# xeTaiz/vit-tf

Measured on AMD Instinct MI355X. Metric: slices/sec (ViT-S/8, 512^3 vol: feature volume + 16-query similarity), higher is better.
Workload: dtype fp16; 1 GPU; 512^3 CT-like synthetic volume (seed 0), ViT-S/8, fos 64: 1536 slices of 512x512 (N=4097) per step + 16-query similarity -> the metric's configuration (BASELINE configs[2]); engine_batch=512, weights=seeded synthetic vits8 (seed 0), parallelism=single GPU

## Files before the change

include/vittf.h:

```cpp
#ifndef VITTF_H
#define VITTF_H

#include <stddef.h>
#include <stdint.h>

#ifdef __cplusplus
extern "C" {
#endif

#define VITTF_ABI_VERSION 6

typedef enum vittf_status {
  VITTF_OK = 0,
  VITTF_ERR_INVALID_ARG = -1,
  VITTF_ERR_WORKSPACE = -2,
  VITTF_ERR_LAUNCH = -3,
  VITTF_ERR_NO_DEVICE = -4
} vittf_status;

typedef enum vittf_dtype { VITTF_BF16 = 0, VITTF_FP16 = 1 } vittf_dtype;

typedef enum vittf_axis { VITTF_AXIS_X = 0, VITTF_AXIS_Y = 1, VITTF_AXIS_Z = 2 } vittf_axis;

typedef enum vittf_sample_mode { VITTF_SAMPLE_NEAREST = 0, VITTF_SAMPLE_TRILINEAR = 1 } vittf_sample_mode;

int vittf_abi_version(void);
const char* vittf_status_string(int status);
int vittf_device_count(void);

typedef struct vittf_vit_config {
  int32_t embed_dim;
  int32_t depth;
  int32_t heads;
  int32_t patch;
  int32_t dtype;
  float   ln_eps;
  int32_t attention_fp8;
  int32_t flags;
} vittf_vit_config;
enum {
  VITTF_CFG_SEPARATE_LN = 1,
  VITTF_CFG_UNSCALED_Q = 2,
  VITTF_CFG_FP8_HEAD_SCALES = 4
};
#define VITTF_MAX_REGISTER_TOKENS 8
#define VITTF_TAIL_STEPS 112

typedef struct vittf_vit_weights {
  const float* pe_w_t;
  const float* pe_b;
  const void*  qkv_w;
  const float* qkv_b;
  const void*  proj_w;
  const float* proj_b;
  const void*  fc1_w;
  const float* fc1_b;
  const void*  fc2_w;
  const float* fc2_b;
  const void*  tail_packed;
  const void*  qkv_packed;
  const float* ln1_g;
  const float* ln1_b;
  const float* ln2_g;
  const float* ln2_b;
} vittf_vit_weights;

typedef struct vittf_pos_embed {
  const float* cls_plus_pos0;
  const float* patch_pos;
} vittf_pos_embed;

typedef struct vittf_slice_view {
  const float* vol;
  int64_t stride_slice;
  int64_t stride_row;
  int64_t stride_col;
  int32_t in_rows;
  int32_t in_cols;
  int32_t out_rows;
  int32_t out_cols;
  const float* minmax;
} vittf_slice_view;

size_t vittf_minmax_workspace_bytes(void);
int vittf_volume_minmax(const float* vol, int64_t n, float* out_minmax, void* ws, size_t ws_bytes, void* stream);

size_t vittf_vit_workspace_bytes(const vittf_vit_config* cfg, int32_t batch, int32_t tokens);

int vittf_vit_k_features(const vittf_vit_config* cfg, const vittf_vit_weights* w, const vittf_pos_embed* pos,
                         const vittf_slice_view* view, int32_t slice0, int32_t batch, int32_t qkv_part,
                         uint16_t* k_out, void* ws, size_t ws_bytes, void* stream);

int vittf_vit_qkv_features(const vittf_vit_config* cfg, const vittf_vit_weights* w, const vittf_pos_embed* pos,
                           const vittf_slice_view* view, int32_t slice0, int32_t batch, int32_t part_mask,
                           uint16_t* q_out, uint16_t* k_out, uint16_t* v_out, void* ws, size_t ws_bytes, void* stream);

int vittf_vit_qkv_features_reg(const vittf_vit_config* cfg, const vittf_vit_weights* w, const vittf_pos_embed* pos,
                               const vittf_slice_view* view, int32_t slice0, int32_t batch, int32_t part_mask,
                               const float* reg_rows, int32_t n_reg, uint16_t* q_out, uint16_t* k_out, uint16_t* v_out,
                               void* ws, size_t ws_bytes, void* stream);

typedef struct vittf_rope_table {
  const float* cos;
  const float* sin;
  int32_t patches;
} vittf_rope_table;

int vittf_vit_qkv_features_rope(const vittf_vit_config* cfg, const vittf_vit_weights* w, const vittf_pos_embed* pos,
                                const vittf_slice_view* view, int32_t slice0, int32_t batch, int32_t part_mask,
                                const float* reg_rows, int32_t n_reg, const vittf_rope_table* table, uint16_t* q_out,
                                uint16_t* k_out, uint16_t* v_out, void* ws, size_t ws_bytes, void* stream);

int vittf_vit_features(const vittf_vit_config* cfg, const vittf_vit_weights* w, const vittf_pos_embed* pos,
                       const vittf_slice_view* view, int32_t slice0, int32_t batch, int32_t part_mask, const float* reg_rows,
                       int32_t n_reg, const vittf_rope_table* table, const float* norm_g, const float* norm_b, uint16_t* q_out,
                       uint16_t* k_out, uint16_t* v_out, uint16_t* t_out, void* ws, size_t ws_bytes, void* stream);

typedef enum vittf_kernel_class {
  VITTF_KERNEL_PATCH_EMBED = 0, VITTF_KERNEL_LAYERNORM = 1,
  VITTF_KERNEL_GEMM = 2,
  VITTF_KERNEL_ATTENTION = 3, VITTF_KERNEL_MLP = 4,
  VITTF_KERNEL_GEMM_QKV = 5,
  VITTF_KERNEL_GEMM_PROJ = 6,
  VITTF_KERNEL_GEMM_FC1 = 7,
  VITTF_KERNEL_GEMM_FC2 = 8,
  VITTF_KERNEL_SIMILARITY = 9,
  VITTF_KERNEL_CLASSES = 10
} vittf_kernel_class;
int vittf_profiler_enable(int32_t class_mask);
int vittf_profiler_collect(double* ms_per_class, int64_t* launches_per_class);
const char* vittf_profiler_kernel_name(int32_t kernel_class);


int vittf_patch_embed(const vittf_vit_config* cfg, const vittf_vit_weights* w, const vittf_pos_embed* pos,
                      const vittf_slice_view* view, int32_t slice0, int32_t batch, float* tokens_out, void* stream);

int vittf_patch_embed_reg(const vittf_vit_config* cfg, const vittf_vit_weights* w, const vittf_pos_embed* pos,
                          const vittf_slice_view* view, int32_t slice0, int32_t batch, const float* reg_rows, int32_t n_reg,
                          float* tokens_out, void* stream);

int vittf_layernorm(const float* x, const float* g, const float* b, void* y, int64_t rows, int32_t d,
                    float eps, int32_t dtype, void* stream);

int vittf_token_features(const float* x, const float* norm_g, const float* norm_b, uint16_t* t_out, int32_t batch,
                         int32_t tokens, int32_t prefix, int32_t d, float eps, void* stream);

typedef enum vittf_epilogue {
  VITTF_EPI_BIAS = 0,
  VITTF_EPI_BIAS_GELU = 1,
  VITTF_EPI_BIAS_RESIDUAL = 2,
  VITTF_EPI_KFEAT = 3,
  VITTF_EPI_BIAS_QKV = 4
} vittf_epilogue;

int vittf_gemm(const void* a, const void* w, const float* bias, void* out, int64_t rows, int32_t n, int32_t k,
               int32_t epilogue, int32_t tokens, int32_t dtype, void* stream);

int vittf_gemm_kfeat_parts(const void* a, const void* w, const float* bias, int64_t rows, int32_t d, int32_t k,
                           int32_t tokens, int32_t part_mask, void* q_out, void* k_out, void* v_out, int32_t dtype,
                           void* stream);

int vittf_gemm_kfeat_parts_reg(const void* a, const void* w, const float* bias, int64_t rows, int32_t d, int32_t k,
                               int32_t tokens, int32_t n_reg, int32_t part_mask, void* q_out, void* k_out, void* v_out,
                               int32_t dtype, void* stream);

int vittf_gemm_residual_ln(const void* a, const void* w, const float* bias, float* x, int64_t rows, int32_t n, int32_t k,
                           int32_t dtype, const float* ln_g, const float* ln_b, float ln_eps, void* h, void* stream);

size_t vittf_gemm_as_workspace_bytes(void);
int vittf_gemm_as(const void* a, const void* w_packed, const float* bias, void* out, int64_t rows, int32_t n, int32_t k,
                  int32_t epilogue, int32_t dtype, void* tile_counter, void* stream);

size_t vittf_block_tail_workspace_bytes(void);
int vittf_block_tail(const void* attn_out, const void* w_packed, const float* proj_b, const float* ln2_g, const float* ln2_b,
                     const float* b1, const float* b2, float* x, int64_t rows, int32_t d, int32_t dtype, const float* ln_g,
                     const float* ln_b, float ln_eps, void* h_out, void* tile_counter, void* stream);

int vittf_rope_qk(void* qkv, int64_t rows, int32_t tokens, int32_t prefix, int32_t heads, const vittf_rope_table* table,
                  int32_t dtype, void* stream);

int vittf_attention(const void* qkv, void* out, int32_t batch, int32_t tokens, int32_t heads, int32_t dtype,
                    int32_t q_prescaled, void* stream);

int64_t vittf_attention_rescale_count(int32_t reset);

size_t vittf_attention_fp8_workspace_bytes(int32_t batch, int32_t tokens, int32_t heads);
int vittf_attention_fp8(const void* qkv, void* out, int32_t batch, int32_t tokens, int32_t heads, int32_t dtype, void* ws,
                        size_t ws_bytes, void* stream);

int vittf_gemm_qkv_fp8(const void* a, const void* w, const float* bias, void* qkv_out, int64_t rows, int32_t n, int32_t k,
                       int32_t tokens, int32_t heads, int32_t dtype, void* ws, size_t ws_bytes, void* stream);
int vittf_attention_fp8_rows(const void* qkv, void* out, int32_t batch, int32_t tokens, int32_t heads, int32_t dtype, void* ws,
                             size_t ws_bytes, void* stream);


int vittf_pool_slices(const uint16_t* k_slices, int32_t k_slice0, int32_t k_nslices, int32_t total_slices,
                      int32_t n_out, int32_t win0, int32_t nwin, int32_t f0, int32_t f1, int32_t d,
                      uint16_t* dst, int64_t dst_stride_d, int64_t dst_stride_win, int64_t dst_stride_row,
                      int64_t dst_stride_col, void* stream);

int vittf_pool_slices3d(const uint16_t* k_slices, int32_t k_slice0, int32_t k_nslices, int32_t total_slices,
                        int32_t n_out, int32_t win0, int32_t nwin, int32_t f0, int32_t f1, int32_t d,
                        uint16_t* dst, int64_t dst_stride_d, int64_t dst_stride_win, int64_t dst_stride_row,
                        int64_t dst_stride_col, int32_t o0, int32_t o1, int32_t slice_dim, void* stream);

int vittf_assemble_sum(const uint16_t* gz, const uint16_t* gy, const uint16_t* gx, int32_t nranks,
                       const int32_t chunk[3], int32_t d, int32_t n0, int32_t n1, int32_t n2, uint16_t* out,
                       void* stream);


int vittf_sample_features(const void* feat, int32_t feat_is_fp16, int32_t f, int32_t n0, int32_t n1, int32_t n2,
                          const float* rel, int32_t a, int32_t mode, const float* voxel_norm, float* out, void* stream);

int vittf_voxel_norm(const uint16_t* feat, int32_t f, int64_t nvox, float* out, void* stream);

size_t vittf_similarity_workspace_bytes(int32_t classes, int64_t nvox, int32_t annotations);

int vittf_similarity(const uint16_t* feat, int32_t f, int32_t n0, int32_t n1, int32_t n2, const float* qf,
                     const int32_t* class_start_host, int32_t classes, int32_t big_a_mean, const float* voxel_norm,
                     int32_t o0, int32_t o1, int32_t o2, uint8_t* out, void* ws, size_t ws_bytes, void* stream);

#define VITTF_QUERY_MAX_A 64
size_t vittf_similarity_query_workspace_bytes(int32_t classes, int64_t nvox, int32_t annotations, int32_t f);
int vittf_similarity_query(const uint16_t* feat, int32_t f, int32_t n0, int32_t n1, int32_t n2, const float* rel_host,
                           const int32_t* class_start_host, int32_t classes, int32_t big_a_mean, const float* voxel_norm,
                           int32_t o0, int32_t o1, int32_t o2, uint8_t* out, void* ws, size_t ws_bytes, void* stream);

int vittf_similarity_maps_f32(const void* feat, int32_t feat_is_fp16, int32_t f, int32_t n0, int32_t n1, int32_t n2,
                              const float* qf, const int32_t* class_start_host, int32_t classes, int32_t mode,
                              float exponent, const float* voxel_norm, float* maps_out, void* ws, size_t ws_bytes,
                              void* stream);

int vittf_topk_voxels(const float* maps, int32_t nmaps, int64_t nvox, int32_t k, int32_t* idx_out, void* stream);

int vittf_mean_pairwise_distance(const float* x, int32_t n, int32_t f, int32_t measure, float* dist, void* stream);

#define VITTF_GRAM_RUN 2048
#define VITTF_PCA_MAX_K 64

size_t vittf_feature_gram_workspace_bytes(int32_t f, int64_t nvox);
int vittf_feature_gram(const uint16_t* feat, int32_t f, int64_t nvox, double* gram, double* sums, void* ws, size_t ws_bytes,
                       void* stream);

int vittf_feature_project(const uint16_t* feat, int32_t f, int64_t nvox, const float* comp, const float* offset, int32_t k,
                          uint16_t* out, void* stream);

#define VITTF_KMEANS_MAX_C 64

int vittf_kmeans_assign(const uint16_t* feat, int32_t f, int64_t nvox, const float* cent, const float* half_sq, int32_t c,
                        uint8_t* labels, float* best, void* stream);

size_t vittf_kmeans_sums_workspace_bytes(int32_t f, int64_t nvox, int32_t c);
int vittf_kmeans_sums(const uint16_t* feat, int32_t f, int64_t nvox, const uint8_t* labels, int32_t c, double* sums,
                      int64_t* counts, void* ws, size_t ws_bytes, void* stream);

#define VITTF_SVM_MAX_CLASSES 8
#define VITTF_SVM_MAX_SV 65536

size_t vittf_svm_rbf_workspace_bytes(int32_t f, int32_t n_sv, int32_t classes);
int vittf_svm_rbf_decide(const uint16_t* feat, int32_t f, int64_t nvox, const uint16_t* sv, const float* pair_coef,
                         const float* intercept, int32_t n_sv, int32_t classes, float gamma, const float* voxel_norm,
                         uint8_t* labels, float* decision, void* ws, size_t ws_bytes, void* stream);

int vittf_svm_linear_decide(const uint16_t* feat, int32_t f, int64_t nvox, const float* w, const float* intercept,
                            int32_t classes, const float* voxel_norm, uint8_t* labels, float* decision, void* stream);

#define VITTF_FOREST_MAX_CLASSES 8
#define VITTF_FOREST_MAX_TREES 4096
#define VITTF_FOREST_MAX_NODES 65535
#define VITTF_FOREST_MAX_DEPTH 64
int vittf_forest_decide(const uint16_t* feat, int32_t f, int64_t nvox, const uint32_t* nodes, const uint16_t* leaf_values,
                        const uint32_t* tree_offset, int32_t trees, int32_t classes, int32_t max_depth, uint8_t* labels,
                        uint32_t* votes, void* stream);

#define VITTF_MLP_MAX_CLASSES 8
#define VITTF_MLP_MAX_LAYERS 2
#define VITTF_MLP_MAX_WIDTH 256
size_t vittf_mlp_workspace_bytes(int32_t f, const int32_t* widths, int32_t layers, int32_t classes);
int vittf_mlp_decide(const uint16_t* feat, int32_t f, int64_t nvox, const float* weights, const float* biases,
                     const int32_t* widths, int32_t layers, int32_t classes, const float* voxel_norm, uint8_t* labels,
                     float* logits, uint8_t* probs, void* workspace, size_t workspace_bytes, void* stream);

#define VITTF_KNN_MAX_K 32
#define VITTF_KNN_MAX_CLASSES 8
#define VITTF_KNN_MAX_BANK 65536
size_t vittf_knn_workspace_bytes(int32_t f, int32_t n_bank);
int vittf_knn_decide(const uint16_t* feat, int32_t f, int64_t nvox, const uint16_t* bank, const uint8_t* bank_class,
                     int32_t n_bank, int32_t classes, int32_t k, float inv_temperature, const float* voxel_norm,
                     uint8_t* labels, float* scores, int32_t* nn_index, float* nn_sim, void* ws, size_t ws_bytes,
                     void* stream);

#define VITTF_VOXFEAT_CHANNELS 11
size_t vittf_voxel_feature_stats_workspace_bytes(int32_t n0, int32_t n1, int32_t n2);
int vittf_voxel_feature_stats(const float* vol, int32_t n0, int32_t n1, int32_t n2, float vmax, double* stats, void* ws,
                              size_t ws_bytes, void* stream);
int vittf_voxel_features(const float* vol, int32_t n0, int32_t n1, int32_t n2, float vmax, const double* stats, int32_t channels,
                         const int64_t* voxel_index, int64_t v0, int64_t n, uint16_t* out, int64_t out_stride, void* stream);

int vittf_erode_mask(const uint8_t* src, int32_t n0, int32_t n1, int32_t n2, int32_t class_id, int32_t connectivity,
                     uint8_t* dst, void* stream);

size_t vittf_surface_shell_workspace_bytes(int32_t n0, int32_t n1, int32_t n2);
int vittf_surface_shell(const uint8_t* labels, int32_t n0, int32_t n1, int32_t n2, int32_t class_id, int32_t connectivity,
                        uint8_t* shell, void* ws, size_t ws_bytes, void* stream);

int vittf_confusion_matrix(const uint8_t* target, const uint8_t* pred, int64_t n, int32_t classes, int64_t* counts,
                           void* stream);

#define VITTF_CC_TILE0 4
#define VITTF_CC_TILE1 8
#define VITTF_CC_TILE2 64
size_t vittf_components_workspace_bytes(int32_t n0, int32_t n1, int32_t n2);
int vittf_label_components(const uint8_t* src, int32_t n0, int32_t n1, int32_t n2, int32_t select, int32_t connectivity,
                           int32_t* labels, void* ws, size_t ws_bytes, void* stream);

int vittf_component_sizes(const int32_t* labels, int64_t nvox, int32_t* sizes, void* stream);

int vittf_filter_components(const uint8_t* src, const int32_t* labels, const int32_t* sizes, int64_t nvox, int32_t min_size,
                            int32_t keep_label, int32_t fill, uint8_t* dst, void* stream);

#define VITTF_EDT_MAX_DIM 2048
#define VITTF_EDT_NO_SITE 2147483647
size_t vittf_edt_workspace_bytes(int32_t n0, int32_t n1, int32_t n2);
int vittf_edt_sq(const uint8_t* src, int32_t n0, int32_t n1, int32_t n2, int32_t value, int32_t mode, int32_t* d2_out,
                 int32_t* site_out, void* ws, size_t ws_bytes, void* stream);
int vittf_edt_sq_weighted(const uint8_t* src, int32_t n0, int32_t n1, int32_t n2, int32_t value, int32_t mode,
                          const double* w2_host, float* d2_out, int32_t* site_out, void* ws, size_t ws_bytes, void* stream);

#define VITTF_RENDER_MAX_DIM 2048
#define VITTF_RENDER_MAX_IMAGE 8192
#define VITTF_RENDER_MAX_CLASSES 8
int vittf_render_prepare(const float* volume, int64_t nvox, double vmin, double vmax, uint16_t* q, void* stream);
size_t vittf_render_occupancy_bytes(int32_t n0, int32_t n1, int32_t n2);
int vittf_render_occupancy(const uint16_t* q, int32_t n0, int32_t n1, int32_t n2, const float* table, const uint8_t* maps,
                           int32_t classes, int32_t m0, int32_t m1, int32_t m2, const int32_t* lo_host, uint8_t* occ,
                           void* stream);
int vittf_render(const uint16_t* q, int32_t n0, int32_t n1, int32_t n2, const float* spacing_host, const float* table,
                 const uint8_t* maps, int32_t classes, int32_t m0, int32_t m1, int32_t m2, const int32_t* lo_host,
                 const int32_t* hi_host, const float* class_rgbs_host, const uint8_t* occ, const float* camera_host,
                 int32_t width, int32_t height, float dt, const float* shade_host, float* rgba_out, void* stream);

int vittf_resize_nearest_u8(const uint8_t* src, int32_t n0, int32_t n1, int32_t n2, uint8_t* dst, int32_t o0, int32_t o1,
                            int32_t o2, int32_t equals, void* stream);

int vittf_widen_f16(const uint16_t* src, int64_t n, float* dst, void* stream);

typedef struct vittf_bilateral_params {
  double sigma_spatial;
  double lam;
  double a_diag_min;
  double cg_tol;
  int32_t cg_maxiter;
  int32_t bistochastize_iters;
  int32_t pad;
  float crop_threshold;
} vittf_bilateral_params;

size_t vittf_bilateral_workspace_bytes(int32_t o0, int32_t o1, int32_t o2, double sigma_spatial, int32_t luma_bins);

int vittf_bilateral_refine(const float* sim_in, int32_t n0, int32_t n1, int32_t n2, const float* volume, int32_t v0,
                           int32_t v1, int32_t v2, int32_t o0, int32_t o1, int32_t o2, const int32_t* luma_bin_host,
                           int32_t luma_bins, const vittf_bilateral_params* prm, float* sim_out, int32_t* info_host,
                           void* ws, size_t ws_bytes, void* stream);

int vittf_quantize_wrap_u8(const float* sim, int64_t n, uint8_t* out, float* max_scratch, void* stream);

int vittf_assign_labels(const uint8_t* sims, int32_t classes, int64_t n, const int32_t* thr_host, uint8_t* labels,
                        void* stream);

#ifdef __cplusplus
}
#endif
#endif
```

vit-tf_amd/_lib.py:

```python
import ctypes as C
import os

_HERE = os.path.dirname(os.path.abspath(__file__))
LIB_PATH = os.path.join(_HERE, 'libvittf.so')

BF16, FP16 = 0, 1
DTYPES = {'bf16': BF16, 'bfloat16': BF16, 'fp16': FP16, 'float16': FP16, 'half': FP16}
SAMPLE_MODES = {'nearest': 0, 'bilinear': 1, 'trilinear': 1}
EPI_BIAS, EPI_BIAS_GELU, EPI_BIAS_RESIDUAL, EPI_KFEAT, EPI_BIAS_QKV = 0, 1, 2, 3, 4


class VitConfig(C.Structure):
    _fields_ = [('embed_dim', C.c_int32), ('depth', C.c_int32), ('heads', C.c_int32), ('patch', C.c_int32),
                ('dtype', C.c_int32), ('ln_eps', C.c_float), ('attention_fp8', C.c_int32), ('flags', C.c_int32)]


CFG_SEPARATE_LN, CFG_UNSCALED_Q, CFG_FP8_HEAD_SCALES = 1, 2, 4


class VitWeights(C.Structure):
    _fields_ = [(n, C.c_void_p) for n in (
        'pe_w_t', 'pe_b', 'qkv_w', 'qkv_b', 'proj_w', 'proj_b', 'fc1_w', 'fc1_b', 'fc2_w', 'fc2_b', 'tail_packed', 'qkv_packed',
        'ln1_g', 'ln1_b', 'ln2_g', 'ln2_b')]


class PosEmbed(C.Structure):
    _fields_ = [('cls_plus_pos0', C.c_void_p), ('patch_pos', C.c_void_p)]


class RopeTable(C.Structure):
    _fields_ = [('cos', C.c_void_p), ('sin', C.c_void_p), ('patches', C.c_int32)]


class SliceView(C.Structure):
    _fields_ = [('vol', C.c_void_p), ('stride_slice', C.c_int64), ('stride_row', C.c_int64),
                ('stride_col', C.c_int64), ('in_rows', C.c_int32), ('in_cols', C.c_int32),
                ('out_rows', C.c_int32), ('out_cols', C.c_int32), ('minmax', C.c_void_p)]


class VittfError(RuntimeError):
    pass


class BilateralParams(C.Structure):
    _fields_ = [('sigma_spatial', C.c_double), ('lam', C.c_double), ('a_diag_min', C.c_double), ('cg_tol', C.c_double),
                ('cg_maxiter', C.c_int32), ('bistochastize_iters', C.c_int32), ('pad', C.c_int32),
                ('crop_threshold', C.c_float)]


_vp, _i32, _i64, _sz = C.c_void_p, C.c_int32, C.c_int64, C.c_size_t
_P = C.POINTER

SIGNATURES = {
    'vittf_abi_version': (C.c_int, []),
    'vittf_status_string': (C.c_char_p, [C.c_int]),
    'vittf_device_count': (C.c_int, []),
    'vittf_minmax_workspace_bytes': (_sz, []),
    'vittf_volume_minmax': (C.c_int, [_vp, _i64, _vp, _vp, _sz, _vp]),
    'vittf_vit_workspace_bytes': (_sz, [_P(VitConfig), _i32, _i32]),
    'vittf_vit_k_features': (C.c_int, [_P(VitConfig), _P(VitWeights), _P(PosEmbed), _P(SliceView), _i32, _i32, _i32,
                                       _vp, _vp, _sz, _vp]),
    'vittf_vit_qkv_features': (C.c_int, [_P(VitConfig), _P(VitWeights), _P(PosEmbed), _P(SliceView), _i32, _i32, _i32,
                                         _vp, _vp, _vp, _vp, _sz, _vp]),
    'vittf_vit_qkv_features_reg': (C.c_int, [_P(VitConfig), _P(VitWeights), _P(PosEmbed), _P(SliceView), _i32, _i32, _i32,
                                             _vp, _i32, _vp, _vp, _vp, _vp, _sz, _vp]),
    'vittf_vit_qkv_features_rope': (C.c_int, [_P(VitConfig), _P(VitWeights), _P(PosEmbed), _P(SliceView), _i32, _i32, _i32,
                                              _vp, _i32, _P(RopeTable), _vp, _vp, _vp, _vp, _sz, _vp]),
    'vittf_vit_features': (C.c_int, [_P(VitConfig), _P(VitWeights), _P(PosEmbed), _P(SliceView), _i32, _i32, _i32, _vp, _i32,
                                     _P(RopeTable), _vp, _vp, _vp, _vp, _vp, _vp, _vp, _sz, _vp]),
    'vittf_profiler_enable': (C.c_int, [_i32]),
    'vittf_profiler_collect': (C.c_int, [_P(C.c_double), _P(_i64)]),
    'vittf_profiler_kernel_name': (C.c_char_p, [_i32]),
    'vittf_patch_embed': (C.c_int, [_P(VitConfig), _P(VitWeights), _P(PosEmbed), _P(SliceView), _i32, _i32, _vp, _vp]),
    'vittf_patch_embed_reg': (C.c_int, [_P(VitConfig), _P(VitWeights), _P(PosEmbed), _P(SliceView), _i32, _i32, _vp, _i32, _vp,
                                        _vp]),
    'vittf_token_features': (C.c_int, [_vp, _vp, _vp, _vp, _i32, _i32, _i32, _i32, C.c_float, _vp]),
    'vittf_layernorm': (C.c_int, [_vp, _vp, _vp, _vp, _i64, _i32, C.c_float, _i32, _vp]),
    'vittf_gemm': (C.c_int, [_vp, _vp, _vp, _vp, _i64, _i32, _i32, _i32, _i32, _i32, _vp]),
    'vittf_gemm_kfeat_parts': (C.c_int, [_vp, _vp, _vp, _i64, _i32, _i32, _i32, _i32, _vp, _vp, _vp, _i32, _vp]),
    'vittf_gemm_kfeat_parts_reg': (C.c_int, [_vp, _vp, _vp, _i64, _i32, _i32, _i32, _i32, _i32, _vp, _vp, _vp, _i32, _vp]),
    'vittf_gemm_residual_ln': (C.c_int, [_vp, _vp, _vp, _vp, _i64, _i32, _i32, _i32, _vp, _vp, C.c_float, _vp, _vp]),
    'vittf_block_tail_workspace_bytes': (_sz, []),
    'vittf_block_tail': (C.c_int, [_vp, _vp, _vp, _vp, _vp, _vp, _vp, _vp, _i64, _i32, _i32, _vp, _vp, C.c_float, _vp, _vp, _vp]),
    'vittf_gemm_as_workspace_bytes': (_sz, []),
    'vittf_gemm_as': (C.c_int, [_vp, _vp, _vp, _vp, _i64, _i32, _i32, _i32, _i32, _vp, _vp]),
    'vittf_rope_qk': (C.c_int, [_vp, _i64, _i32, _i32, _i32, _P(RopeTable), _i32, _vp]),
    'vittf_attention': (C.c_int, [_vp, _vp, _i32, _i32, _i32, _i32, _i32, _vp]),
    'vittf_attention_rescale_count': (_i64, [_i32]),
    'vittf_attention_fp8_workspace_bytes': (_sz, [_i32, _i32, _i32]),
    'vittf_attention_fp8': (C.c_int, [_vp, _vp, _i32, _i32, _i32, _i32, _vp, _sz, _vp]),
    'vittf_gemm_qkv_fp8': (C.c_int, [_vp, _vp, _vp, _vp, _i64, _i32, _i32, _i32, _i32, _i32, _vp, _sz, _vp]),
    'vittf_attention_fp8_rows': (C.c_int, [_vp, _vp, _i32, _i32, _i32, _i32, _vp, _sz, _vp]),
    'vittf_pool_slices': (C.c_int, [_vp, _i32, _i32, _i32, _i32, _i32, _i32, _i32, _i32, _i32, _vp, _i64, _i64, _i64,
                                    _i64, _vp]),
    'vittf_pool_slices3d': (C.c_int, [_vp, _i32, _i32, _i32, _i32, _i32, _i32, _i32, _i32, _i32, _vp, _i64, _i64, _i64,
                                      _i64, _i32, _i32, _i32, _vp]),
    'vittf_assemble_sum': (C.c_int, [_vp, _vp, _vp, _i32, _P(_i32), _i32, _i32, _i32, _i32, _vp, _vp]),
    'vittf_sample_features': (C.c_int, [_vp, _i32, _i32, _i32, _i32, _i32, _vp, _i32, _i32, _vp, _vp, _vp]),
    'vittf_voxel_norm': (C.c_int, [_vp, _i32, _i64, _vp, _vp]),
    'vittf_similarity_workspace_bytes': (_sz, [_i32, _i64, _i32]),
    'vittf_similarity': (C.c_int, [_vp, _i32, _i32, _i32, _i32, _vp, _P(_i32), _i32, _i32, _vp, _i32, _i32, _i32, _vp, _vp,
                                   _sz, _vp]),
    'vittf_similarity_query_workspace_bytes': (_sz, [_i32, _i64, _i32, _i32]),
    'vittf_similarity_query': (C.c_int, [_vp, _i32, _i32, _i32, _i32, _P(C.c_float), _P(_i32), _i32, _i32, _vp, _i32, _i32, _i32,
                                         _vp, _vp, _sz, _vp]),
    'vittf_similarity_maps_f32': (C.c_int, [_vp, _i32, _i32, _i32, _i32, _i32, _vp, _P(_i32), _i32, _i32, C.c_float, _vp, _vp,
                                            _vp, _sz, _vp]),
    'vittf_feature_gram_workspace_bytes': (_sz, [_i32, _i64]),
    'vittf_feature_gram': (C.c_int, [_vp, _i32, _i64, _vp, _vp, _vp, _sz, _vp]),
    'vittf_feature_project': (C.c_int, [_vp, _i32, _i64, _vp, _vp, _i32, _vp, _vp]),
    'vittf_kmeans_assign': (C.c_int, [_vp, _i32, _i64, _vp, _vp, _i32, _vp, _vp, _vp]),
    'vittf_kmeans_sums_workspace_bytes': (_sz, [_i32, _i64, _i32]),
    'vittf_kmeans_sums': (C.c_int, [_vp, _i32, _i64, _vp, _i32, _vp, _vp, _vp, _sz, _vp]),
    'vittf_svm_rbf_workspace_bytes': (_sz, [_i32, _i32, _i32]),
    'vittf_svm_rbf_decide': (C.c_int, [_vp, _i32, _i64, _vp, _vp, _vp, _i32, _i32, C.c_float, _vp, _vp, _vp, _vp, _sz, _vp]),
    'vittf_svm_linear_decide': (C.c_int, [_vp, _i32, _i64, _vp, _vp, _i32, _vp, _vp, _vp, _vp]),
    'vittf_forest_decide': (C.c_int, [_vp, _i32, _i64, _vp, _vp, _vp, _i32, _i32, _i32, _vp, _vp, _vp]),
    'vittf_mlp_workspace_bytes': (_sz, [_i32, _P(_i32), _i32, _i32]),
    'vittf_mlp_decide': (C.c_int, [_vp, _i32, _i64, _vp, _vp, _P(_i32), _i32, _i32, _vp, _vp, _vp, _vp, _vp, _sz, _vp]),
    'vittf_knn_workspace_bytes': (_sz, [_i32, _i32]),
    'vittf_knn_decide': (C.c_int, [_vp, _i32, _i64, _vp, _vp, _i32, _i32, _i32, C.c_float, _vp, _vp, _vp, _vp, _vp, _vp, _sz, _vp]),
    'vittf_voxel_feature_stats_workspace_bytes': (_sz, [_i32, _i32, _i32]),
    'vittf_voxel_feature_stats': (C.c_int, [_vp, _i32, _i32, _i32, C.c_float, _vp, _vp, _sz, _vp]),
    'vittf_voxel_features': (C.c_int, [_vp, _i32, _i32, _i32, C.c_float, _vp, _i32, _vp, _i64, _i64, _vp, _i64, _vp]),
    'vittf_topk_voxels':(C.c_int, [_vp, _i32, _i64, _i32, _vp, _vp]),
    'vittf_mean_pairwise_distance': (C.c_int, [_vp, _i32, _i32, _i32, _vp, _vp]),
    'vittf_erode_mask': (C.c_int, [_vp, _i32, _i32, _i32, _i32, _i32, _vp, _vp]),
    'vittf_surface_shell_workspace_bytes': (_sz, [_i32, _i32, _i32]),
    'vittf_surface_shell': (C.c_int, [_vp, _i32, _i32, _i32, _i32, _i32, _vp, _vp, _sz, _vp]),
    'vittf_confusion_matrix': (C.c_int, [_vp, _vp, _i64, _i32, _vp, _vp]),
    'vittf_components_workspace_bytes': (_sz, [_i32, _i32, _i32]),
    'vittf_label_components': (C.c_int, [_vp, _i32, _i32, _i32, _i32, _i32, _vp, _vp, _sz, _vp]),
    'vittf_component_sizes': (C.c_int, [_vp, _i64, _vp, _vp]),
    'vittf_filter_components': (C.c_int, [_vp, _vp, _vp, _i64, _i32, _i32, _i32, _vp, _vp]),
    'vittf_edt_workspace_bytes': (_sz, [_i32, _i32, _i32]),
    'vittf_edt_sq': (C.c_int, [_vp, _i32, _i32, _i32, _i32, _i32, _vp, _vp, _vp, _sz, _vp]),
    'vittf_edt_sq_weighted': (C.c_int, [_vp, _i32, _i32, _i32, _i32, _i32, _P(C.c_double), _vp, _vp, _vp, _sz, _vp]),
    'vittf_render_prepare': (C.c_int, [_vp, _i64, C.c_double, C.c_double, _vp, _vp]),
    'vittf_render_occupancy_bytes': (_sz, [_i32, _i32, _i32]),
    'vittf_render_occupancy': (C.c_int, [_vp, _i32, _i32, _i32, _vp, _vp, _i32, _i32, _i32, _i32, _P(_i32), _vp, _vp]),
    'vittf_render': (C.c_int, [_vp, _i32, _i32, _i32, _P(C.c_float), _vp, _vp, _i32, _i32, _i32, _i32, _P(_i32), _P(_i32),
                               _P(C.c_float), _vp, _P(C.c_float), _i32, _i32, C.c_float, _P(C.c_float), _vp, _vp]),
    'vittf_resize_nearest_u8': (C.c_int, [_vp, _i32, _i32, _i32, _vp, _i32, _i32, _i32, _i32, _vp]),
    'vittf_widen_f16': (C.c_int, [_vp, _i64, _vp, _vp]),
    'vittf_bilateral_workspace_bytes': (_sz, [_i32, _i32, _i32, C.c_double, _i32]),
    'vittf_bilateral_refine': (C.c_int, [_vp, _i32, _i32, _i32, _vp, _i32, _i32, _i32, _i32, _i32, _i32, _P(_i32), _i32,
                                         _P(BilateralParams), _vp, _P(_i32), _vp, _sz, _vp]),
    'vittf_quantize_wrap_u8': (C.c_int, [_vp, _i64, _vp, _vp, _vp]),
    'vittf_assign_labels': (C.c_int, [_vp, _i32, _i64, _P(_i32), _vp, _vp]),
}

_lib = None


def load():
    global _lib
    if _lib is not None:
        return _lib
    if not os.path.exists(LIB_PATH):
        raise VittfError(
            f'{LIB_PATH} not found: the HIP library has not been built. Run '
            f'`python -c "import __graft_entry__ as g; g.build()"` (or `make -C vit-tf_amd/csrc`) first. '
            'There is no CPU fallback for this path.')
    lib = C.CDLL(LIB_PATH)
    for name, (res, args) in SIGNATURES.items():
        fn = getattr(lib, name)
        fn.restype, fn.argtypes = res, args
    if lib.vittf_abi_version() != ABI_VERSION:
        raise VittfError('libvittf.so ABI version mismatch; rebuild it')
    _lib = lib
    return lib


KERNEL_CLASSES = ('patch_embed', 'layernorm', 'gemm', 'attention', 'mlp', 'gemm_qkv', 'gemm_proj', 'gemm_fc1', 'gemm_fc2',
                  'similarity')
ABI_VERSION = 6
MAX_REGISTER_TOKENS = 8
QUERY_MAX_A = 64
GRAM_RUN = 2048
PCA_MAX_K = 64
KMEANS_MAX_C = 64
CC_TILE = (4, 8, 64)
SVM_MAX_CLASSES = 8
SVM_MAX_SV = 65536
FOREST_MAX_CLASSES = 8
FOREST_MAX_TREES = 4096
FOREST_MAX_NODES = 65535
FOREST_MAX_DEPTH = 64
MLP_MAX_CLASSES = 8
MLP_MAX_LAYERS = 2
MLP_MAX_WIDTH = 256
KNN_MAX_K = 32
KNN_MAX_CLASSES = 8
KNN_MAX_BANK = 65536
EDT_MAX_DIM = 2048
EDT_NO_SITE = 2 ** 31 - 1
RENDER_MAX_DIM = 2048
RENDER_MAX_IMAGE = 8192
RENDER_MAX_CLASSES = 8
VOXFEAT_CHANNELS = 11
KMEANS_SPANS = 128


def profiler_enable(on=True, classes=None):
    mask = 0
    if on:
        mask = -1 if classes is None else sum(1 << KERNEL_CLASSES.index(c) for c in classes)
    check(load().vittf_profiler_enable(mask), 'vittf_profiler_enable')


def kernel_name(kernel_class):
    return load().vittf_profiler_kernel_name(KERNEL_CLASSES.index(kernel_class)).decode()


def profiler_collect():
    ms = (C.c_double * len(KERNEL_CLASSES))()
    n = (C.c_int64 * len(KERNEL_CLASSES))()
    check(load().vittf_profiler_collect(ms, n), 'vittf_profiler_collect')
    return {k: (ms[i], n[i]) for i, k in enumerate(KERNEL_CLASSES)}


def check(rc, what=''):
    if rc != 0:
        msg = load().vittf_status_string(rc).decode()
        raise VittfError(f'{what or "vittf call"} failed: {msg} ({rc})')


def require_device():
    import torch
    lib = load()
    if not torch.cuda.is_available():
        raise VittfError('no GPU visible to PyTorch-ROCm: the vit-tf hot path runs only on MI355X (gfx950); '
                         'there is no CPU fallback')
    return lib


def stream_ptr():
    import torch
    return C.c_void_p(torch.cuda.current_stream().cuda_stream)


def ptr(t):
    return None if t is None else C.c_void_p(t.data_ptr())
```

vit-tf_amd/csrc/engine.hip:

```cpp
#include "vittf_internal.h"

#include <stdlib.h>
#include <vector>

namespace {
struct ProfRec { hipEvent_t a, b; int cls; };
unsigned g_prof_mask = 0;
std::vector<ProfRec> g_prof_recs;
std::vector<hipEvent_t> g_prof_pool;

hipEvent_t prof_event() {
  if (!g_prof_pool.empty()) { hipEvent_t e = g_prof_pool.back(); g_prof_pool.pop_back(); return e; }
  hipEvent_t e;
  (void)hipEventCreate(&e);
  return e;
}

struct WsLayout {
  size_t x, h, qkv, o, fp8, fp8_bytes, tile_ctr, total;
};

WsLayout ws_layout(int d, int64_t rows, size_t fp8_bytes = 0) {
  const int64_t rp = (rows + 127) / 128 * 128;
  WsLayout l;
  size_t off = 0;
  l.x = off;   off += align256((size_t)rp * d * 4);
  l.h = off;   off += align256((size_t)rp * d * 2);
  l.qkv = off; off += (size_t)rp * 3 * d * 2;
  l.o = off;   off += align256((size_t)rp * d * 2);
  l.fp8 = off; l.fp8_bytes = fp8_bytes; off += align256(fp8_bytes);
  l.tile_ctr = off; off += align256(vittf_block_tail_workspace_bytes());
  l.total = off;
  return l;
}

bool config_ok(const vittf_vit_config* c) {
  return c && c->embed_dim > 0 && c->embed_dim % 128 == 0 && c->embed_dim <= 1024 && c->depth >= 1 &&
         c->heads * 64 == c->embed_dim && (c->patch == 8 || c->patch == 14 || c->patch == 16) &&
         (c->dtype == VITTF_BF16 || c->dtype == VITTF_FP16) && c->ln_eps > 0.f;
}
}

void* vittf_prof_begin(int cls, void* stream) {
  if (!((g_prof_mask >> cls) & 1u)) return nullptr;
  ProfRec* r = new ProfRec;
  r->cls = cls; r->a = prof_event(); r->b = prof_event();
  (void)hipEventRecord(r->a, (hipStream_t)stream);
  return r;
}
void vittf_prof_end(void* token, void* stream) {
  ProfRec* r = (ProfRec*)token;
  (void)hipEventRecord(r->b, (hipStream_t)stream);
  g_prof_recs.push_back(*r);
  delete r;
}

extern "C" int vittf_abi_version(void) { return VITTF_ABI_VERSION; }

extern "C" const char* vittf_status_string(int status) {
  switch (status) {
    case VITTF_OK: return "ok";
    case VITTF_ERR_INVALID_ARG: return "invalid argument";
    case VITTF_ERR_WORKSPACE: return "workspace too small";
    case VITTF_ERR_LAUNCH: return "HIP launch error";
    case VITTF_ERR_NO_DEVICE: return "no gfx950 device";
    default: return "unknown status";
  }
}

extern "C" int vittf_device_count(void) {
  int n = 0;
  if (hipGetDeviceCount(&n) != hipSuccess) return 0;
  int ok = 0;
  for (int i = 0; i < n; ++i) {
    hipDeviceProp_t p;
    if (hipGetDeviceProperties(&p, i) == hipSuccess && __builtin_strstr(p.gcnArchName, "gfx950")) ++ok;
  }
  return ok;
}

extern "C" size_t vittf_vit_workspace_bytes(const vittf_vit_config* cfg, int32_t batch, int32_t tokens) {
  if (!config_ok(cfg) || batch <= 0 || tokens <= 1) return 0;
  return ws_layout(cfg->embed_dim, (int64_t)batch * tokens,
                   cfg->attention_fp8 ? vittf_attention_fp8_workspace_bytes(batch, tokens, cfg->heads) : 0).total;
}

extern "C" int vittf_vit_features(const vittf_vit_config* cfg, const vittf_vit_weights* w, const vittf_pos_embed* pos,
                                  const vittf_slice_view* view, int32_t slice0, int32_t batch, int32_t part_mask,
                                  const float* reg_rows, int32_t n_reg, const vittf_rope_table* rope, const float* norm_g,
                                  const float* norm_b, uint16_t* q_out, uint16_t* k_out, uint16_t* v_out, uint16_t* t_out,
                                  void* ws, size_t ws_bytes, void* stream) {
  if (!config_ok(cfg) || !w || !pos || !view || !ws || batch <= 0 || slice0 < 0) return VITTF_ERR_INVALID_ARG;
  if (n_reg < 0 || n_reg > VITTF_MAX_REGISTER_TOKENS || (n_reg > 0 && !reg_rows)) return VITTF_ERR_INVALID_ARG;
  if (rope && (cfg->attention_fp8 || !rope->cos || !rope->sin)) return VITTF_ERR_INVALID_ARG;
  if (part_mask <= 0 || part_mask > 15) return VITTF_ERR_INVALID_ARG;
  if (((part_mask & 1) && !q_out) || ((part_mask & 2) && !k_out) || ((part_mask & 4) && !v_out)) return VITTF_ERR_INVALID_ARG;
  const bool want_t = (part_mask & 8) != 0;
  if (want_t && (!t_out || !norm_g || !norm_b)) return VITTF_ERR_INVALID_ARG;
  if (!w->qkv_w || !w->qkv_b || !w->proj_w || !w->proj_b || !w->fc1_w || !w->fc1_b || !w->fc2_w || !w->fc2_b ||
      !w->ln1_g || !w->ln1_b || !w->ln2_g || !w->ln2_b)
    return VITTF_ERR_INVALID_ARG;
  const int d = cfg->embed_dim, p = cfg->patch, L = cfg->depth, dt = cfg->dtype;
  if (view->out_rows % p || view->out_cols % p) return VITTF_ERR_INVALID_ARG;
  const int tokens = (view->out_rows / p) * (view->out_cols / p) + 1 + n_reg;
  const int64_t rows = (int64_t)batch * tokens;
  if (rope && rope->patches != tokens - 1 - n_reg) return VITTF_ERR_INVALID_ARG;
  if (rows * (int64_t)((d == 384 && w->tail_packed) ? 3 * d : 4 * d) > 0xffffffffll) return VITTF_ERR_INVALID_ARG;
  const WsLayout lay = ws_layout(d, rows, cfg->attention_fp8 ? vittf_attention_fp8_workspace_bytes(batch, tokens, cfg->heads) : 0);
  if (ws_bytes < lay.total) return VITTF_ERR_WORKSPACE;
  if (((uintptr_t)ws & 255) != 0) return VITTF_ERR_INVALID_ARG;
  char* base = (char*)ws;
  float* X = (float*)(base + lay.x);
  void* H = base + lay.h;
  void* QKV = base + lay.qkv;
  void* O = base + lay.o;
  void* G = QKV;

  int rc;
  { ProfScope ps(VITTF_KERNEL_PATCH_EMBED, stream); rc = vittf_patch_embed_reg(cfg, w, pos, view, slice0, batch, reg_rows, n_reg, X, stream); }
  if (rc) return rc;
  const size_t esz = 2;
  const bool res_ln = !(cfg->flags & VITTF_CFG_SEPARATE_LN) && (d == 384 || d == 768);
  const int pre = (cfg->flags & VITTF_CFG_UNSCALED_Q) ? 0 : 1;
  const bool fp8_rows = !(cfg->flags & VITTF_CFG_FP8_HEAD_SCALES) && cfg->attention_fp8 && pre && d >= 768 && d % 256 == 0;
  const bool tail = d == 384 && w->tail_packed && res_ln;
  const bool qkv_as = d == 384 && w->qkv_packed && !cfg->attention_fp8;
  for (int l = 0; l < L; ++l) {
    const char* qkv_w = (const char*)w->qkv_w + (size_t)l * 3 * d * d * esz;
    if (res_ln ? l == 0 : true) {
      ProfScope ps(VITTF_KERNEL_LAYERNORM, stream);
      rc = vittf_layernorm(X, w->ln1_g + (size_t)l * d, w->ln1_b + (size_t)l * d, H, rows, d, cfg->ln_eps, dt, stream);
      if (rc) return rc;
    }
    if (l == L - 1 && (part_mask & 7)) {
      ProfScope ps(VITTF_KERNEL_GEMM, stream);
      rc = vittf_gemm_kfeat_parts_reg(H, qkv_w, w->qkv_b + (size_t)l * 3 * d, rows, d, d, tokens, n_reg, part_mask & 7, q_out,
                                      k_out, v_out, dt, stream);
      if (rc || !want_t) return rc;
    }
    const float* next_g = l == L - 1 ? norm_g : w->ln1_g + (size_t)(l + 1) * d;
    const float* next_b = l == L - 1 ? norm_b : w->ln1_b + (size_t)(l + 1) * d;
    { ProfScope ps(VITTF_KERNEL_GEMM_QKV, stream);
      if (fp8_rows)
        rc = vittf_gemm_qkv_fp8(H, qkv_w, w->qkv_b + (size_t)l * 3 * d, QKV, rows, 3 * d, d, tokens, cfg->heads, dt,
                                base + lay.fp8, lay.fp8_bytes, stream);
      else if (qkv_as)
        rc = vittf_gemm_as(H, (const char*)w->qkv_packed + (size_t)l * 3 * d * d * esz, w->qkv_b + (size_t)l * 3 * d, QKV, rows, 3 * d, d,
                           pre ? VITTF_EPI_BIAS_QKV : VITTF_EPI_BIAS, dt, base + lay.tile_ctr, stream);
      else
        rc = vittf_gemm(H, qkv_w, w->qkv_b + (size_t)l * 3 * d, QKV, rows, 3 * d, d,
                        pre ? VITTF_EPI_BIAS_QKV : VITTF_EPI_BIAS, 0, dt, stream);
      if (!rc && rope) rc = vittf_rope_qk(QKV, rows, tokens, 1 + n_reg, cfg->heads, rope, dt, stream); }
    if (rc) return rc;
    { ProfScope ps(VITTF_KERNEL_ATTENTION, stream);
      if (fp8_rows)
        rc = vittf_attention_fp8_rows(QKV, O, batch, tokens, cfg->heads, dt, base + lay.fp8, lay.fp8_bytes, stream);
      else if (cfg->attention_fp8 && pre)
        rc = vittf_attention_fp8(QKV, O, batch, tokens, cfg->heads, dt, base + lay.fp8, lay.fp8_bytes, stream);
      else
        rc = vittf_attention(QKV, O, batch, tokens, cfg->heads, dt, pre, stream); }
    if (rc) return rc;
    if (tail) {
      ProfScope ps(VITTF_KERNEL_MLP, stream);
      rc = vittf_block_tail(O, (const char*)w->tail_packed + (size_t)l * VITTF_TAIL_STEPS * 12288 * esz, w->proj_b + (size_t)l * d,
                            w->ln2_g + (size_t)l * d, w->ln2_b + (size_t)l * d, w->fc1_b + (size_t)l * 4 * d,
                            w->fc2_b + (size_t)l * d, X, rows, d, dt, next_g, next_b, cfg->ln_eps, H, base + lay.tile_ctr,
                            stream);
      if (rc) return rc;
      continue;
    }
    { ProfScope ps(VITTF_KERNEL_GEMM_PROJ, stream);
      if (res_ln)
        rc = vittf_gemm_residual_ln(O, (const char*)w->proj_w + (size_t)l * d * d * esz, w->proj_b + (size_t)l * d, X, rows, d,
                                    d, dt, w->ln2_g + (size_t)l * d, w->ln2_b + (size_t)l * d, cfg->ln_eps, H, stream);
      else
        rc = vittf_gemm(O, (const char*)w->proj_w + (size_t)l * d * d * esz, w->proj_b + (size_t)l * d, X, rows, d, d,
                        VITTF_EPI_BIAS_RESIDUAL, 0, dt, stream); }
    if (rc) return rc;
    if (!res_ln) {
      ProfScope ps(VITTF_KERNEL_LAYERNORM, stream);
      rc = vittf_layernorm(X, w->ln2_g + (size_t)l * d, w->ln2_b + (size_t)l * d, H, rows, d, cfg->ln_eps, dt, stream);
      if (rc) return rc;
    }
    { ProfScope ps(VITTF_KERNEL_GEMM_FC1, stream);
      rc = vittf_gemm(H, (const char*)w->fc1_w + (size_t)l * 4 * d * d * esz, w->fc1_b + (size_t)l * 4 * d, G, rows,
                      4 * d, d, VITTF_EPI_BIAS_GELU, 0, dt, stream); }
    if (rc) return rc;
    { ProfScope ps(VITTF_KERNEL_GEMM_FC2, stream);
      if (res_ln)
        rc = vittf_gemm_residual_ln(G, (const char*)w->fc2_w + (size_t)l * 4 * d * d * esz, w->fc2_b + (size_t)l * d, X, rows,
                                    d, 4 * d, dt, next_g, next_b, cfg->ln_eps, H, stream);
      else
        rc = vittf_gemm(G, (const char*)w->fc2_w + (size_t)l * 4 * d * d * esz, w->fc2_b + (size_t)l * d, X, rows, d,
                        4 * d, VITTF_EPI_BIAS_RESIDUAL, 0, dt, stream); }
    if (rc) return rc;
  }
  ProfScope ps(VITTF_KERNEL_LAYERNORM, stream);
  return vittf_token_features(X, norm_g, norm_b, t_out, batch, tokens, 1 + n_reg, d, cfg->ln_eps, stream);
}

extern "C" int vittf_vit_qkv_features_rope(const vittf_vit_config* cfg, const vittf_vit_weights* w, const vittf_pos_embed* pos,
                                           const vittf_slice_view* view, int32_t slice0, int32_t batch, int32_t part_mask,
                                           const float* reg_rows, int32_t n_reg, const vittf_rope_table* rope, uint16_t* q_out,
                                           uint16_t* k_out, uint16_t* v_out, void* ws, size_t ws_bytes, void* stream) {
  if (part_mask <= 0 || part_mask > 7) return VITTF_ERR_INVALID_ARG;
  return vittf_vit_features(cfg, w, pos, view, slice0, batch, part_mask, reg_rows, n_reg, rope, nullptr, nullptr, q_out, k_out,
                            v_out, nullptr, ws, ws_bytes, stream);
}

extern "C" int vittf_vit_qkv_features_reg(const vittf_vit_config* cfg, const vittf_vit_weights* w, const vittf_pos_embed* pos,
                                          const vittf_slice_view* view, int32_t slice0, int32_t batch, int32_t part_mask,
                                          const float* reg_rows, int32_t n_reg, uint16_t* q_out, uint16_t* k_out,
                                          uint16_t* v_out, void* ws, size_t ws_bytes, void* stream) {
  return vittf_vit_qkv_features_rope(cfg, w, pos, view, slice0, batch, part_mask, reg_rows, n_reg, nullptr, q_out, k_out, v_out, ws,
                                     ws_bytes, stream);
}

extern "C" int vittf_vit_qkv_features(const vittf_vit_config* cfg, const vittf_vit_weights* w, const vittf_pos_embed* pos,
                                      const vittf_slice_view* view, int32_t slice0, int32_t batch, int32_t part_mask,
                                      uint16_t* q_out, uint16_t* k_out, uint16_t* v_out, void* ws, size_t ws_bytes,
                                      void* stream) {
  return vittf_vit_qkv_features_reg(cfg, w, pos, view, slice0, batch, part_mask, nullptr, 0, q_out, k_out, v_out, ws, ws_bytes,
                                    stream);
}

extern "C" int vittf_vit_k_features(const vittf_vit_config* cfg, const vittf_vit_weights* w, const vittf_pos_embed* pos,
                                    const vittf_slice_view* view, int32_t slice0, int32_t batch, int32_t qkv_part,
                                    uint16_t* k_out, void* ws, size_t ws_bytes, void* stream) {
  if (!k_out || qkv_part < 0 || qkv_part > 2) return VITTF_ERR_INVALID_ARG;
  uint16_t* outs[3] = {nullptr, nullptr, nullptr};
  outs[qkv_part] = k_out;
  return vittf_vit_qkv_features(cfg, w, pos, view, slice0, batch, 1 << qkv_part, outs[0], outs[1], outs[2], ws, ws_bytes,
                                stream);
}

static const char* g_kernel_names[VITTF_KERNEL_CLASSES] = {};
void vittf_note_kernel(int cls, const char* name) {
  if (cls >= 0 && cls < VITTF_KERNEL_CLASSES) g_kernel_names[cls] = name;
}
extern "C" const char* vittf_profiler_kernel_name(int32_t cls) {
  return (cls >= 0 && cls < VITTF_KERNEL_CLASSES && g_kernel_names[cls]) ? g_kernel_names[cls] : "";
}

extern "C" int vittf_profiler_enable(int32_t on) {
  for (auto& r : g_prof_recs) { g_prof_pool.push_back(r.a); g_prof_pool.push_back(r.b); }
  g_prof_recs.clear();
  g_prof_mask = (unsigned)on;
  return VITTF_OK;
}

extern "C" int vittf_profiler_collect(double* ms_per_class, int64_t* launches_per_class) {
  if (!ms_per_class || !launches_per_class) return VITTF_ERR_INVALID_ARG;
  for (int i = 0; i < VITTF_KERNEL_CLASSES; ++i) { ms_per_class[i] = 0.0; launches_per_class[i] = 0; }
  for (auto& r : g_prof_recs) {
    if (hipEventSynchronize(r.b) != hipSuccess) return VITTF_ERR_LAUNCH;
    float ms = 0.f;
    if (hipEventElapsedTime(&ms, r.a, r.b) != hipSuccess) return VITTF_ERR_LAUNCH;
    ms_per_class[r.cls] += ms;
    launches_per_class[r.cls] += 1;
  }
  return VITTF_OK;
}
```

vit-tf_amd/csrc/frontend.hip:

```cpp
#include "vittf_common.h"

namespace {

constexpr int MM_BLOCKS = 1024;

__device__ __forceinline__ void wave_minmax(float& lo, float& hi) {
#pragma unroll
  for (int off = 32; off > 0; off >>= 1) {
    lo = fminf(lo, __shfl_xor(lo, off));
    hi = fmaxf(hi, __shfl_xor(hi, off));
  }
}

__device__ __forceinline__ void block_minmax(float& lo, float& hi) {
  __shared__ float s_lo[4], s_hi[4];
  wave_minmax(lo, hi);
  const int wave = threadIdx.x >> 6, lane = threadIdx.x & 63;
  if (lane == 0) { s_lo[wave] = lo; s_hi[wave] = hi; }
  __syncthreads();
  lo = fminf(fminf(s_lo[0], s_lo[1]), fminf(s_lo[2], s_lo[3]));
  hi = fmaxf(fmaxf(s_hi[0], s_hi[1]), fmaxf(s_hi[2], s_hi[3]));
}

__global__ __launch_bounds__(256) void minmax_partial(const float* __restrict__ v, int64_t n, float* __restrict__ part) {
  float lo = INFINITY, hi = -INFINITY;
  const int64_t n4 = n >> 2;
  const float4* v4 = reinterpret_cast<const float4*>(v);
  for (int64_t i = (int64_t)blockIdx.x * 256 + threadIdx.x; i < n4; i += (int64_t)gridDim.x * 256) {
    const float4 x = v4[i];
    lo = fminf(fminf(lo, x.x), fminf(fminf(x.y, x.z), x.w));
    hi = fmaxf(fmaxf(hi, x.x), fmaxf(fmaxf(x.y, x.z), x.w));
  }
  if (blockIdx.x == 0)
    for (int64_t i = (n4 << 2) + threadIdx.x; i < n; i += 256) { lo = fminf(lo, v[i]); hi = fmaxf(hi, v[i]); }
  block_minmax(lo, hi);
  if (threadIdx.x == 0) { part[2 * blockIdx.x] = lo; part[2 * blockIdx.x + 1] = hi; }
}

__global__ __launch_bounds__(256) void minmax_final(const float* __restrict__ part, int nblocks, float* __restrict__ out) {
  float lo = INFINITY, hi = -INFINITY;
  for (int i = threadIdx.x; i < nblocks; i += 256) { lo = fminf(lo, part[2 * i]); hi = fmaxf(hi, part[2 * i + 1]); }
  block_minmax(lo, hi);
  if (threadIdx.x == 0) { out[0] = lo; out[1] = hi; }
}

constexpr int TP = 32;

template <int P>
__global__ __launch_bounds__(384) void patch_embed_kernel(vittf_slice_view view, int slice0, const float* __restrict__ w_t,
                                                          const float* __restrict__ bias,
                                                          const float* __restrict__ cls_pos0,
                                                          const float* __restrict__ patch_pos, float* __restrict__ tokens_out,
                                                          int d, int f0, int f1, int nreg, const float* __restrict__ reg_rows) {
  constexpr int PP = P * P;
  __shared__ __attribute__((aligned(16))) float px[TP][PP + 4];
  const int npatch = f0 * f1;
  const int tokens = npatch + 1 + nreg;
  const int b = blockIdx.y;
  const int p0 = blockIdx.x * TP;
  const float lo = view.minmax[0], hi = view.minmax[1];
  const float range = hi - lo;
  const float sr = (float)view.in_rows / (float)view.out_rows;
  const float sc = (float)view.in_cols / (float)view.out_cols;
  const float* slice = view.vol + (int64_t)(slice0 + b) * view.stride_slice;

  for (int e = threadIdx.x; e < TP * PP; e += blockDim.x) {
    const int pl = e / PP, k = e - pl * PP;
    const int p = p0 + pl;
    float v = 0.f;
    if (p < npatch) {
      const int py = p / f1, pxx = p - py * f1;
      const int iy = py * P + k / P, ix = pxx * P + k % P;
      int ry = (int)floorf((float)iy * sr);
      int cx = (int)floorf((float)ix * sc);
      ry = ry < view.in_rows - 1 ? ry : view.in_rows - 1;
      cx = cx < view.in_cols - 1 ? cx : view.in_cols - 1;
      const float raw = slice[(int64_t)ry * view.stride_row + (int64_t)cx * view.stride_col];
      v = (raw - lo) / range;
    }
    px[pl][k] = v;
  }
  __syncthreads();

  float* out_b = tokens_out + (int64_t)b * tokens * d;
  float* out_p = out_b + (int64_t)nreg * d;
  for (int dd = threadIdx.x; dd < d; dd += blockDim.x) {
    float acc[TP];
#pragma unroll
    for (int i = 0; i < TP; ++i) acc[i] = 0.f;
    for (int k = 0; k < PP; k += 4) {
      const float w0 = w_t[(int64_t)k * d + dd], w1 = w_t[(int64_t)(k + 1) * d + dd];
      const float w2 = w_t[(int64_t)(k + 2) * d + dd], w3 = w_t[(int64_t)(k + 3) * d + dd];
#pragma unroll
      for (int i = 0; i < TP; ++i) {
        const float4 v = *reinterpret_cast<const float4*>(&px[i][k]);
        acc[i] = fmaf(v.x, w0, acc[i]);
        acc[i] = fmaf(v.y, w1, acc[i]);
        acc[i] = fmaf(v.z, w2, acc[i]);
        acc[i] = fmaf(v.w, w3, acc[i]);
      }
    }
    const float bv = bias[dd];
#pragma unroll
    for (int i = 0; i < TP; ++i) {
      const int p = p0 + i;
      if (p < npatch) out_p[(int64_t)(1 + p) * d + dd] = acc[i] + bv + patch_pos[(int64_t)p * d + dd];
    }
  }
  if (blockIdx.x == 0)
    for (int e = threadIdx.x; e < (1 + nreg) * d; e += blockDim.x) out_b[e] = e < d ? cls_pos0[e] : reg_rows[e - d];
}

constexpr int PEM_D = 384, PEM_K = 64, PEM_FRAGS = (PEM_D / 32) * (PEM_K / 16) * 2;
__global__ __launch_bounds__(512, 1) void patch_embed_mfma_kernel(vittf_slice_view view, int slice0, int batch,
                                                                  const float* __restrict__ w_t, const float* __restrict__ bias,
                                                                  const float* __restrict__ cls_pos0,
                                                                  const float* __restrict__ patch_pos,
                                                                  float* __restrict__ tokens_out, int f0, int f1, int nreg,
                                                                  const float* __restrict__ reg_rows) {
  __shared__ __attribute__((aligned(16))) unsigned short wlds[PEM_FRAGS * 512];
  const int tid = threadIdx.x, lane = tid & 63, wave = tid >> 6;
  const int h = lane >> 5, l31 = lane & 31;
  for (int it = tid; it < (PEM_FRAGS / 2) * 64; it += 512) {
    const int fr = it >> 6, ln = it & 63;
    const int ot = fr >> 2, s = fr & 3;
    const int i = ln & 31, hh = ln >> 5;
#pragma unroll
    for (int e = 0; e < 8; ++e) {
      const float v = w_t[(int64_t)(16 * s + 8 * hh + e) * PEM_D + 32 * ot + i];
      const unsigned short hi = f32_to_f16bits(v);
      const unsigned short lo = f32_to_f16bits(v - f16bits_to_f32(hi));
      wlds[((fr * 2 + 0) * 64 + ln) * 8 + e] = hi;
      wlds[((fr * 2 + 1) * 64 + ln) * 8 + e] = lo;
    }
  }
  __syncthreads();
  const int npatch = f0 * f1, tokens = npatch + 1 + nreg;
  const int64_t rows = (int64_t)batch * tokens;
  const float lo_v = view.minmax[0], range = view.minmax[1] - view.minmax[0];
  const float sr = (float)view.in_rows / (float)view.out_rows;
  const float sc = (float)view.in_cols / (float)view.out_cols;
  const int64_t ntile = (rows + 255) / 256;
  for (int64_t tile = blockIdx.x; tile < ntile; tile += gridDim.x) {
    const int64_t r = tile * 256 + wave * 32 + l31;
    const bool valid = r < rows;
    const int b = valid ? (int)(r / tokens) : 0;
    const int t = valid ? (int)(r - (int64_t)b * tokens) : 0;
    const bool patch = valid && t > nreg;
    const int p = patch ? t - 1 - nreg : 0;
    const float* crow = t == 0 ? cls_pos0 : reg_rows + (int64_t)(t - 1) * PEM_D;
    const int py = p / f1, pxx = p - py * f1;
    const float* slice = view.vol + (int64_t)(slice0 + b) * view.stride_slice;
    s16x8_t bh[4], bl[4];
#pragma unroll
    for (int s = 0; s < 4; ++s) {
      const int iy = py * 8 + 2 * s + h;
      int ry = (int)floorf((float)iy * sr);
      ry = ry < view.in_rows - 1 ? ry : view.in_rows - 1;
      unsigned short hi[8], lo[8];
#pragma unroll
      for (int e = 0; e < 8; ++e) {
        const int ix = pxx * 8 + e;
        int cx = (int)floorf((float)ix * sc);
        cx = cx < view.in_cols - 1 ? cx : view.in_cols - 1;
        float v = 0.f;
        if (patch) v = (slice[(int64_t)ry * view.stride_row + (int64_t)cx * view.stride_col] - lo_v) / range;
        hi[e] = f32_to_f16bits(v);
        lo[e] = f32_to_f16bits(v - f16bits_to_f32(hi[e]));
      }
#pragma unroll
      for (int e = 0; e < 8; ++e) { bh[s][e] = (short)hi[e]; bl[s][e] = (short)lo[e]; }
    }
    float* orow = tokens_out + r * PEM_D;
    const float* prow = patch_pos + (int64_t)p * PEM_D;
#pragma unroll 1
    for (int pass = 0; pass < 2; ++pass) {
      f32x16_t acc[6];
#pragma unroll
      for (int j = 0; j < 6; ++j)
#pragma unroll
        for (int q = 0; q < 16; ++q) acc[j][q] = 0.f;
#pragma unroll
      for (int s = 0; s < 4; ++s)
#pragma unroll
        for (int j = 0; j < 6; ++j) {
          const int fr = (6 * pass + j) * 4 + s;
          const s16x8_t ah = *reinterpret_cast<const s16x8_t*>(&wlds[((fr * 2 + 0) * 64 + lane) * 8]);
          const s16x8_t al = *reinterpret_cast<const s16x8_t*>(&wlds[((fr * 2 + 1) * 64 + lane) * 8]);
          acc[j] = mfma32<VITTF_FP16>(ah, bh[s], acc[j]);
          acc[j] = mfma32<VITTF_FP16>(al, bh[s], acc[j]);
          acc[j] = mfma32<VITTF_FP16>(ah, bl[s], acc[j]);
        }
      if (valid) {
#pragma unroll
        for (int j = 0; j < 6; ++j)
#pragma unroll
          for (int g = 0; g < 4; ++g) {
            const int c = 32 * (6 * pass + j) + 8 * g + 4 * h;
            float4 o;
            if (patch) {
              const float4 bv = *reinterpret_cast<const float4*>(bias + c);
              const float4 pv = *reinterpret_cast<const float4*>(prow + c);
              o.x = acc[j][4 * g + 0] + bv.x + pv.x; o.y = acc[j][4 * g + 1] + bv.y + pv.y;
              o.z = acc[j][4 * g + 2] + bv.z + pv.z; o.w = acc[j][4 * g + 3] + bv.w + pv.w;
            } else {
              o = *reinterpret_cast<const float4*>(crow + c);
            }
            *reinterpret_cast<float4*>(orow + c) = o;
          }
      }
    }
  }
}

constexpr int PE14_P = 14, PE14_KS = 14, PE14_GROUPS = 3, PE14_TILES = PEM_D / 32 / PE14_GROUPS;
constexpr int PE14_FRAGS = PE14_TILES * PE14_KS * 2;
__global__ __launch_bounds__(512, 1) void patch_embed14_mfma_kernel(vittf_slice_view view, int slice0, int batch,
                                                                    const float* __restrict__ w_t,
                                                                    const float* __restrict__ bias,
                                                                    const float* __restrict__ cls_pos0,
                                                                    const float* __restrict__ patch_pos,
                                                                    float* __restrict__ tokens_out, int f0, int f1, int nreg,
                                                                    const float* __restrict__ reg_rows) {
  __shared__ __attribute__((aligned(16))) unsigned short wlds[PE14_FRAGS * 512];
  const int tid = threadIdx.x, lane = tid & 63, wave = tid >> 6;
  const int h = lane >> 5, l31 = lane & 31;
  const int grp = blockIdx.x % PE14_GROUPS, wgs = gridDim.x / PE14_GROUPS;
  const int col0 = 32 * PE14_TILES * grp;
  for (int it = tid; it < (PE14_FRAGS / 2) * 64; it += 512) {
    const int fr = it >> 6, ln = it & 63;
    const int ot = fr / PE14_KS, s = fr - ot * PE14_KS;
    const int i = ln & 31, hh = ln >> 5;
#pragma unroll
    for (int e = 0; e < 8; ++e) {
      const int kc = 8 * hh + e;
      const float v = kc < PE14_P ? w_t[(int64_t)(PE14_P * s + kc) * PEM_D + col0 + 32 * ot + i] : 0.f;
      const unsigned short hi = f32_to_f16bits(v);
      const unsigned short lo = f32_to_f16bits(v - f16bits_to_f32(hi));
      wlds[((fr * 2 + 0) * 64 + ln) * 8 + e] = hi;
      wlds[((fr * 2 + 1) * 64 + ln) * 8 + e] = lo;
    }
  }
  __syncthreads();
  const int npatch = f0 * f1, tokens = npatch + 1 + nreg;
  const int64_t rows = (int64_t)batch * tokens;
  const float lo_v = view.minmax[0], range = view.minmax[1] - view.minmax[0];
  const float sr = (float)view.in_rows / (float)view.out_rows;
  const float sc = (float)view.in_cols / (float)view.out_cols;
  const int64_t ntile = (rows + 255) / 256;
  for (int64_t tile = blockIdx.x / PE14_GROUPS; tile < ntile; tile += wgs) {
    const int64_t r = tile * 256 + wave * 32 + l31;
    const bool valid = r < rows;
    const int b = valid ? (int)(r / tokens) : 0;
    const int t = valid ? (int)(r - (int64_t)b * tokens) : 0;
    const bool patch = valid && t > nreg;
    const int p = patch ? t - 1 - nreg : 0;
    const float* crow = t == 0 ? cls_pos0 : reg_rows + (int64_t)(t - 1) * PEM_D;
    const int py = p / f1, pxx = p - py * f1;
    const float* slice = view.vol + (int64_t)(slice0 + b) * view.stride_slice;
    int64_t coff[8];
#pragma unroll
    for (int e = 0; e < 8; ++e) {
      const int ix = pxx * PE14_P + 8 * h + e;
      int cx = (int)floorf((float)ix * sc);
      cx = cx < view.in_cols - 1 ? cx : view.in_cols - 1;
      coff[e] = (int64_t)cx * view.stride_col;
    }
    f32x16_t acc[PE14_TILES];
#pragma unroll
    for (int j = 0; j < PE14_TILES; ++j)
#pragma unroll
      for (int q = 0; q < 16; ++q) acc[j][q] = 0.f;
#pragma unroll 2
    for (int s = 0; s < PE14_KS; ++s) {
      const int iy = py * PE14_P + s;
      int ry = (int)floorf((float)iy * sr);
      ry = ry < view.in_rows - 1 ? ry : view.in_rows - 1;
      const float* srow = slice + (int64_t)ry * view.stride_row;
      s16x8_t bh, bl;
#pragma unroll
      for (int e = 0; e < 8; ++e) {
        float v = 0.f;
        if (patch && 8 * h + e < PE14_P) v = (srow[coff[e]] - lo_v) / range;
        const unsigned short hi = f32_to_f16bits(v);
        const unsigned short lo = f32_to_f16bits(v - f16bits_to_f32(hi));
        bh[e] = (short)hi; bl[e] = (short)lo;
      }
#pragma unroll
      for (int j = 0; j < PE14_TILES; ++j) {
        const int fr = j * PE14_KS + s;
        const s16x8_t ah = *reinterpret_cast<const s16x8_t*>(&wlds[((fr * 2 + 0) * 64 + lane) * 8]);
        const s16x8_t al = *reinterpret_cast<const s16x8_t*>(&wlds[((fr * 2 + 1) * 64 + lane) * 8]);
        acc[j] = mfma32<VITTF_FP16>(ah, bh, acc[j]);
        acc[j] = mfma32<VITTF_FP16>(al, bh, acc[j]);
        acc[j] = mfma32<VITTF_FP16>(ah, bl, acc[j]);
      }
    }
    if (valid) {
      float* orow = tokens_out + r * PEM_D;
      const float* prow = patch_pos + (int64_t)p * PEM_D;
#pragma unroll
      for (int j = 0; j < PE14_TILES; ++j)
#pragma unroll
        for (int g = 0; g < 4; ++g) {
          const int c = col0 + 32 * j + 8 * g + 4 * h;
          float4 o;
          if (patch) {
            const float4 bv = *reinterpret_cast<const float4*>(bias + c);
            const float4 pv = *reinterpret_cast<const float4*>(prow + c);
            o.x = acc[j][4 * g + 0] + bv.x + pv.x; o.y = acc[j][4 * g + 1] + bv.y + pv.y;
            o.z = acc[j][4 * g + 2] + bv.z + pv.z; o.w = acc[j][4 * g + 3] + bv.w + pv.w;
          } else {
            o = *reinterpret_cast<const float4*>(crow + c);
          }
          *reinterpret_cast<float4*>(orow + c) = o;
        }
    }
  }
}

}

extern "C" size_t vittf_minmax_workspace_bytes(void) { return 2 * MM_BLOCKS * sizeof(float); }

extern "C" int vittf_volume_minmax(const float* vol, int64_t n, float* out_minmax, void* ws, size_t ws_bytes,
                                   void* stream) {
  if (!vol || !out_minmax || !ws || n <= 0) return VITTF_ERR_INVALID_ARG;
  if (ws_bytes < vittf_minmax_workspace_bytes()) return VITTF_ERR_WORKSPACE;
  if (((uintptr_t)vol & 15) != 0) return VITTF_ERR_INVALID_ARG;
  hipStream_t st = (hipStream_t)stream;
  int64_t want = (n / 4 + 255) / 256;
  const int blocks = (int)(want < 1 ? 1 : (want > MM_BLOCKS ? MM_BLOCKS : want));
  hipLaunchKernelGGL(minmax_partial, dim3(blocks), dim3(256), 0, st, vol, n, (float*)ws);
  hipLaunchKernelGGL(minmax_final, dim3(1), dim3(256), 0, st, (const float*)ws, blocks, out_minmax);
  return vittf_check_launch();
}

extern "C" int vittf_patch_embed_reg(const vittf_vit_config* cfg, const vittf_vit_weights* w, const vittf_pos_embed* pos,
                                     const vittf_slice_view* view, int32_t slice0, int32_t batch, const float* reg_rows,
                                     int32_t n_reg, float* tokens_out, void* stream) {
  if (!cfg || !w || !pos || !view || !tokens_out || batch <= 0 || slice0 < 0) return VITTF_ERR_INVALID_ARG;
  if (n_reg < 0 || n_reg > VITTF_MAX_REGISTER_TOKENS || (n_reg > 0 && !reg_rows)) return VITTF_ERR_INVALID_ARG;
  if (!w->pe_w_t || !w->pe_b || !pos->cls_plus_pos0 || !pos->patch_pos || !view->vol || !view->minmax)
    return VITTF_ERR_INVALID_ARG;
  const int p = cfg->patch;
  if ((p != 8 && p != 14 && p != 16) || view->out_rows % p || view->out_cols % p || view->out_rows <= 0 || view->out_cols <= 0)
    return VITTF_ERR_INVALID_ARG;
  if (view->in_rows <= 0 || view->in_cols <= 0 || batch > 65535) return VITTF_ERR_INVALID_ARG;
  const int f0 = view->out_rows / p, f1 = view->out_cols / p;
  const int nblk = (f0 * f1 + TP - 1) / TP;
  hipStream_t st = (hipStream_t)stream;
  const bool aligned = (((uintptr_t)w->pe_b | (uintptr_t)pos->cls_plus_pos0 | (uintptr_t)pos->patch_pos | (uintptr_t)tokens_out |
                         (n_reg > 0 ? (uintptr_t)reg_rows : 0)) & 15) == 0;
  if (cfg->embed_dim == PEM_D && p == 8 && aligned) {
    const int cus = vittf_current_cus();
    if (cus <= 0) return VITTF_ERR_NO_DEVICE;
    const int64_t ntile = ((int64_t)batch * (f0 * f1 + 1 + n_reg) + 255) / 256;
    vittf_note_kernel(VITTF_KERNEL_PATCH_EMBED, "patch_embed_mfma_kernel");
    hipLaunchKernelGGL(patch_embed_mfma_kernel, dim3((unsigned)(ntile < cus ? ntile : cus)), dim3(512), 0, st, *view, slice0, batch,
                       w->pe_w_t, w->pe_b, pos->cls_plus_pos0, pos->patch_pos, tokens_out, f0, f1, n_reg, reg_rows);
    return vittf_check_launch();
  }
  if (cfg->embed_dim == PEM_D && p == PE14_P && aligned) {
    const int cus = vittf_current_cus();
    if (cus <= 0) return VITTF_ERR_NO_DEVICE;
    const int64_t ntile = ((int64_t)batch * (f0 * f1 + 1 + n_reg) + 255) / 256;
    const int per_group = cus / PE14_GROUPS > 0 ? cus / PE14_GROUPS : 1;
    const int wgs = (int)(ntile < per_group ? ntile : per_group);
    vittf_note_kernel(VITTF_KERNEL_PATCH_EMBED, "patch_embed14_mfma_kernel");
    hipLaunchKernelGGL(patch_embed14_mfma_kernel, dim3((unsigned)(PE14_GROUPS * wgs)), dim3(512), 0, st, *view, slice0, batch,
                       w->pe_w_t, w->pe_b, pos->cls_plus_pos0, pos->patch_pos, tokens_out, f0, f1, n_reg, reg_rows);
    return vittf_check_launch();
  }
  const int threads = cfg->embed_dim % 384 == 0 ? 384 : 256;
  if (p == 8) {
    vittf_note_kernel(VITTF_KERNEL_PATCH_EMBED, "patch_embed_kernel<8>");
    hipLaunchKernelGGL((patch_embed_kernel<8>), dim3(nblk, batch), dim3(threads), 0, st, *view, slice0, w->pe_w_t, w->pe_b,
                       pos->cls_plus_pos0, pos->patch_pos, tokens_out, cfg->embed_dim, f0, f1, n_reg, reg_rows);
  } else if (p == 14) {
    vittf_note_kernel(VITTF_KERNEL_PATCH_EMBED, "patch_embed_kernel<14>");
    hipLaunchKernelGGL((patch_embed_kernel<14>), dim3(nblk, batch), dim3(threads), 0, st, *view, slice0, w->pe_w_t, w->pe_b,
                       pos->cls_plus_pos0, pos->patch_pos, tokens_out, cfg->embed_dim, f0, f1, n_reg, reg_rows);
  } else {
    vittf_note_kernel(VITTF_KERNEL_PATCH_EMBED, "patch_embed_kernel<16>");
    hipLaunchKernelGGL((patch_embed_kernel<16>), dim3(nblk, batch), dim3(threads), 0, st, *view, slice0, w->pe_w_t, w->pe_b,
                       pos->cls_plus_pos0, pos->patch_pos, tokens_out, cfg->embed_dim, f0, f1, n_reg, reg_rows);
  }
  return vittf_check_launch();
}

extern "C" int vittf_patch_embed(const vittf_vit_config* cfg, const vittf_vit_weights* w, const vittf_pos_embed* pos,
                                 const vittf_slice_view* view, int32_t slice0, int32_t batch, float* tokens_out,
                                 void* stream) {
  return vittf_patch_embed_reg(cfg, w, pos, view, slice0, batch, nullptr, 0, tokens_out, stream);
}
```

vit-tf_amd/csrc/tail_fx.hip:

```cpp
#include "vittf_common.h"

#include <type_traits>
#include <utility>

namespace {

constexpr int D = 384, HID = 4 * D, UNITS = HID / 32;
constexpr int SB = 24576, HB = SB / 2;
constexpr int PSTEPS = D / 32;
constexpr int LAG = 4;
constexpr int MSTEPS = 2 * UNITS + LAG;
constexpr int NSEQ = PSTEPS + MSTEPS;
constexpr int NSLOT = 4, AHEAD = NSLOT - 1;
constexpr int PIECES = SB / 1024 / 4;
constexpr int WAIT0 = (AHEAD - 2) * PIECES;
constexpr int NF = 4;
constexpr int PB_OFF = NSLOT * SB;
constexpr int PBH = 4608, PB = 2 * PBH;
constexpr int STG_ROW = 144;
constexpr int AF_SLOT = 1056, AF_H = 528;
constexpr int CONST_OFF = PB_OFF + 4 * PB;
constexpr int C_B1 = 0, C_B2 = HID, C_G1 = HID + D, C_E1 = HID + 2 * D,
              C_BP = HID + 3 * D, C_G2 = HID + 4 * D, C_E2 = HID + 5 * D,
              C_N = HID + 6 * D;
constexpr int NEXT_OFF = CONST_OFF + C_N * 4;
constexpr int LDS_BYTES = NEXT_OFF + 16;
static_assert(LDS_BYTES <= 160 * 1024, "LDS");
static_assert(AHEAD >= 3, "ring depth");
static_assert(32 * STG_ROW <= PBH && 4 * AF_SLOT <= PBH, "pair buffer");

typedef __attribute__((ext_vector_type(4))) unsigned u32x4_t;
typedef __attribute__((ext_vector_type(2))) unsigned u32x2_t;
typedef __attribute__((address_space(3))) const s16x8_t* lds_frag_ptr;
typedef __attribute__((address_space(3))) const f32x4_t* lds_f4_ptr;
typedef __attribute__((address_space(3))) f32x4_t* lds_w4_ptr;
typedef __attribute__((address_space(3))) u32x4_t* lds_wu4_ptr;
typedef __attribute__((address_space(3))) u32x2_t* lds_w2_ptr;
typedef __attribute__((address_space(3))) volatile unsigned* lds_u32_ptr;

struct Ring {
  i32x4_t rsrc;
  unsigned dma_dst;
  int src0;
  int g;
  int slot;
};

__device__ __forceinline__ s16x8_t ld_frag(const unsigned (&base)[4], int f) {
  return *(lds_frag_ptr)(base[f & 3] + (f >> 2) * 4096);
}

__device__ __forceinline__ void lds_dma16_keep(i32x4_t rsrc, unsigned lds_addr, int voff, int soff) {
  asm volatile("s_mov_b32 m0, %0\n\ts_nop 0\n\tbuffer_load_dwordx4 %1, %2, %3 offen lds"
               :: "s"(lds_addr), "v"(voff), "s"(rsrc), "s"(soff) : "memory");
}

struct Gelu3 { float x, p; };
__device__ __forceinline__ void gelu_a(Gelu3& s, float x) {
  s.x = x;
  asm volatile("" : "+v"(s.x));
  s.p = fmaf(-0.000524238159f, fabsf(s.x), 0.00741911121f);
  s.p = fmaf(s.p, fabsf(s.x), -0.0526018888f);
  s.p = fmaf(s.p, fabsf(s.x), -0.459225923f);
  asm volatile("" : "+v"(s.x), "+v"(s.p));
}
__device__ __forceinline__ void gelu_b(Gelu3& s) {
  s.p = fmaf(s.p, fabsf(s.x), -1.15109742f);
  s.p = __builtin_amdgcn_exp2f(fmaf(s.p, fabsf(s.x), -1.0f));
  asm volatile("" : "+v"(s.p));
}
__device__ __forceinline__ float gelu_c(const Gelu3& s) {
  float v = fmaf(-fabsf(s.x), s.p, fmaxf(s.x, 0.f));
  asm volatile("" : "+v"(v));
  return v;
}

template <int WAITN, bool LGKM = false>
__device__ __forceinline__ void x_wait() {
  static_assert(WAITN <= 63, "vmcnt");
  if constexpr (WAITN < 0) {
    if constexpr (LGKM) asm volatile("s_waitcnt lgkmcnt(0)\n\ts_barrier" ::: "memory");
    else asm volatile("s_barrier" ::: "memory");
  } else if constexpr (LGKM) {
    asm volatile("s_waitcnt vmcnt(%0) lgkmcnt(0)\n\ts_barrier" ::"i"(WAITN) : "memory");
  } else {
    asm volatile("s_waitcnt vmcnt(%0)\n\ts_barrier" ::"i"(WAITN) : "memory");
  }
}
template <bool LGKM = false>
__device__ __forceinline__ void sync_wait() {
  if constexpr (LGKM) asm volatile("s_waitcnt lgkmcnt(0)\n\ts_barrier" ::: "memory");
  else asm volatile("s_barrier" ::: "memory");
}

__device__ __forceinline__ int ring_next(const Ring& st) { return st.g + AHEAD < NSEQ ? st.g + AHEAD : st.g + AHEAD - NSEQ; }
__device__ __forceinline__ int ring_free(const Ring& st) { return st.slot == 0 ? NSLOT - 1 : st.slot - 1; }
__device__ __forceinline__ void ring_advance(Ring& st) {
  st.g = st.g + 1 == NSEQ ? 0 : st.g + 1;
  st.slot = st.slot + 1 == NSLOT ? 0 : st.slot + 1;
}
__device__ __forceinline__ void ring_piece(const Ring& st, int i, int g_next, int slot_free) {
  const int off = st.src0 + i * 1024;
  lds_dma16_keep(st.rsrc, st.dma_dst + slot_free * SB + off, (int)((threadIdx.x & 63) * 16), g_next * SB + off);
}
__device__ __forceinline__ void rotate_bases(const Ring& st, unsigned (&base)[4]) {
  const int d_ = st.slot == NSLOT - 1 ? -(NSLOT - 1) * SB : SB;
#pragma unroll
  for (int i = 0; i < 4; ++i) {
    base[i] += d_;
    asm volatile("" : "+v"(base[i]));
  }
}

template <bool LAST, bool DMA, int NM = 12>
__device__ __forceinline__ void ring_gap(const Ring& st, unsigned (&base)[4], s16x8_t (&wf)[NF], int j, int g_next, int slot_free) {
  if (j == NM - NF && !LAST) rotate_bases(st, base);
  if (!(LAST && j >= NM - NF)) wf[j % NF] = ld_frag(base, (j + NF) % NM);
  if (DMA && j % (NM / PIECES) == NM / PIECES - 1) ring_piece(st, j / (NM / PIECES), g_next, slot_free);
}

template <int WAITN, bool LGKM = false>
__device__ __forceinline__ void x_idle_step(Ring& st) {
  x_wait<WAITN, LGKM>();
  const int g_next = ring_next(st), slot_free = ring_free(st);
#pragma unroll
  for (int i = 0; i < PIECES; ++i) ring_piece(st, i, g_next, slot_free);
  ring_advance(st);
}

template <int DT, int KH, bool GELU, bool LAST, bool LGKM>
__device__ __forceinline__ void f_step(Ring& st, unsigned (&base)[4], s16x8_t (&wf)[NF], const s16x8_t (&hf)[D / 16],
                                       f32x16_t& gacc, const f32x16_t& bias_c, const f32x16_t& gprev, u32x4_t& pk) {
  sync_wait<LGKM>();
  Gelu3 s0 = {}, s1 = {};
#pragma unroll
  for (int j = 0; j < 12; ++j) {
    gacc = mfma32<DT>(wf[j % NF], hf[12 * KH + j], (KH == 0 && j == 0) ? bias_c : gacc);
    ring_gap<LAST, false>(st, base, wf, j, 0, 0);
    if constexpr (GELU) {
      const int r = 8 * KH + 2 * (j / 3);
      if (j % 3 == 0) {
        gelu_a(s0, gprev[r]); gelu_a(s1, gprev[r + 1]);
      } else if (j % 3 == 1) {
        gelu_b(s0); gelu_b(s1);
      } else {
        const float v0 = gelu_c(s0), v1 = gelu_c(s1);
        pk[j / 3] = pack2_h16<DT>(v0, v1);
      }
    }
    __builtin_amdgcn_sched_barrier(0);
  }
  ring_advance(st);
}

template <int DT, int OH, bool LAST>
__device__ __forceinline__ void x_step(Ring& st, unsigned (&base)[4], s16x8_t (&wf)[NF], f32x16_t (&xacc)[D / 32],
                                       s16x8_t (&gf)[2], unsigned gf_addr) {
  x_wait<WAIT0>();
  const int g_next = ring_next(st), slot_free = ring_free(st);
  if constexpr (OH == 0) {
    gf[0] = *(lds_frag_ptr)(gf_addr);
    gf[1] = *(lds_frag_ptr)(gf_addr + 1024);
  }
#pragma unroll
  for (int j = 0; j < 12; ++j) {
    xacc[6 * OH + (j >> 1)] = mfma32<DT>(wf[j % NF], gf[j & 1], xacc[6 * OH + (j >> 1)]);
    ring_gap<LAST, true>(st, base, wf, j, g_next, slot_free);
    __builtin_amdgcn_sched_barrier(0);
  }
  ring_advance(st);
}

template <int DT, int WAITN, bool FIRST, bool LAST>
__device__ __forceinline__ void p_step(Ring& st, unsigned (&base)[4], s16x8_t (&wf)[NF], f32x16_t (&xacc)[D / 32],
                                       const s16x8_t (&acur)[2], s16x8_t (&anext)[2], unsigned anext_addr0, unsigned anext_addr1) {
  if constexpr (!FIRST) x_wait<WAITN>();
  const int g_next = ring_next(st), slot_free = ring_free(st);
  if constexpr (!LAST) {
    anext[0] = *(lds_frag_ptr)(anext_addr0);
    anext[1] = *(lds_frag_ptr)(anext_addr1);
  }
#pragma unroll
  for (int j = 0; j < 24; ++j) {
    xacc[j % 12] = mfma32<DT>(wf[j % NF], acur[j / 12], xacc[j % 12]);
    ring_gap<LAST, true, 24>(st, base, wf, j, g_next, slot_free);
    __builtin_amdgcn_sched_barrier(0);
  }
  ring_advance(st);
}

__device__ __forceinline__ constexpr int af_off(int s) { return (((s >> 2) & 1) ? 0 : PBH) + (s & 3) * AF_SLOT; }

struct Ctx {
  const unsigned short* abuf; const unsigned short* wpk; float* x; unsigned short* hout; unsigned* tile_ctr;
  int64_t rows; float ln_eps; int ntiles; int tile; unsigned lds0;
};
__device__ __forceinline__ unsigned uni(unsigned v) { return __builtin_amdgcn_readfirstlane(v); }
template <typename T> __device__ __forceinline__ T* uni_ptr(T* p) {
  const uint64_t v = reinterpret_cast<uint64_t>(p);
  return reinterpret_cast<T*>(((uint64_t)uni((unsigned)(v >> 32)) << 32) | uni((unsigned)v));
}
#define FX_ROLE_ENV                                                                                                       \
  const unsigned short* const abuf = uni_ptr(c.abuf);                                                                     \
  float* const x = uni_ptr(c.x);                                                                                          \
  unsigned short* const hout = uni_ptr(c.hout);                                                                           \
  unsigned* const tile_ctr = uni_ptr(c.tile_ctr);                                                                         \
  const int64_t rows = (int64_t)(((uint64_t)uni((unsigned)((uint64_t)c.rows >> 32)) << 32) | uni((unsigned)c.rows));     \
  const float ln_eps = __uint_as_float(uni(__float_as_uint(c.ln_eps)));                                                   \
  const int ntiles = (int)uni((unsigned)c.ntiles);                                                                        \
  int tile = (int)uni((unsigned)c.tile);                                                                                  \
  const unsigned lds0 = uni(c.lds0);                                                                                      \
  const int tid = threadIdx.x;                                                                                            \
  const int lane = tid & 63, wave = __builtin_amdgcn_readfirstlane(tid >> 6);                                             \
  const int rb = wave & 3;                                                                                                \
  const int h = lane >> 5, l31 = lane & 31;                                                                               \
  unsigned cl = lds0 + CONST_OFF + 16 * h;                                                                                \
  asm volatile("" : "+v"(cl));                                                                                            \
  auto cst4 = [&](int i) { return *(lds_f4_ptr)(cl + 4 * i); };             \
  const unsigned nxt = lds0 + NEXT_OFF;                                                                                   \
  Ring st;                                                                                                                \
  st.rsrc = lds_dma_rsrc(uni_ptr(c.wpk), (unsigned)(NSEQ * SB));                                                          \
  st.src0 = rb * (PIECES * 1024);                                                                                         \
  st.dma_dst = lds0;                                                                                                      \
  st.g = 0;                                                                                                               \
  st.slot = 0;                                                                                                            \
  const int aoff0 = tile_off(l31, h);                                                                                     \
  const unsigned pbuf = lds0 + PB_OFF + rb * PB;                           \
   \
  auto tile_rsrc = [&](const void* p, int64_t tile, int row_bytes) {                                                      \
    const int64_t first = tile * 128, left = rows - first;                                                                \
    const int nrows = tile < 0 || left <= 0 || !p ? 0 : left < 128 ? (int)left : 128;                                     \
    return __builtin_amdgcn_make_buffer_rsrc(const_cast<char*>(reinterpret_cast<const char*>(p)) + (nrows ? first : 0) * row_bytes, 0, \
                                             nrows * row_bytes, 0x00020000);                                              \
  };                                                                                                                      \
  (void)abuf; (void)x; (void)hout; (void)tile_ctr; (void)ln_eps; (void)ntiles; (void)l31; (void)aoff0; (void)nxt; (void)cst4; (void)tile_rsrc

template <int DT>
__device__ __attribute__((noinline)) void run_f(Ctx c) {
  FX_ROLE_ENV;
  asm volatile("s_setprio 3");
  unsigned pbl = pbuf + lane * 16;
  asm volatile("" : "+v"(pbl));
  u32x4_t fb[48];
  const int q8 = lane >> 3, c8 = lane & 7;
  __amdgpu_buffer_rsrc_t ra, rx;
  const int ao = (rb * 32 + q8) * (D * 2) + c8 * 16, xo = (rb * 32 + q8) * (D * 4) + c8 * 16;
  auto load_a = [&](int cg) {
#pragma unroll
    for (int i = 0; i < 4; ++i) fb[4 * cg + i] = __builtin_amdgcn_raw_buffer_load_b128(ra, ao + cg * 128, i * 8 * (D * 2), 0);
  };
  auto load_chunk = [&](int c) {
    const int r0 = c < 6 ? 24 + 4 * c : 4 * (c - 6);
#pragma unroll
    for (int i = 0; i < 4; ++i) fb[r0 + i] = __builtin_amdgcn_raw_buffer_load_b128(rx, xo + c * 128, i * 8 * (D * 4), 0);
  };
  const unsigned af_wr = pbuf + (c8 >> 1) * AF_SLOT + (c8 & 1) * AF_H + q8 * 16;
  auto put_a = [&](int cg) {
#pragma unroll
    for (int i = 0; i < 4; ++i) *(lds_wu4_ptr)(af_wr + af_off(4 * cg) + i * 128) = fb[4 * cg + i];
  };
  const unsigned ch_wr = pbuf + q8 * STG_ROW + c8 * 16;
  auto put_chunk = [&](int c) {
    const int r0 = c < 6 ? 24 + 4 * c : 4 * (c - 6);
#pragma unroll
    for (int i = 0; i < 4; ++i) *(lds_wu4_ptr)(ch_wr + (c & 1) * PBH + i * 8 * STG_ROW) = fb[r0 + i];
  };
  auto fetch_rows = [&](int t) {
    ra = tile_rsrc(abuf, t, D * 2);
    rx = tile_rsrc(x, t, D * 4);
#pragma unroll
    for (int cg = 0; cg < 6; ++cg) load_a(cg);
#pragma unroll
    for (int c = 0; c < 6; ++c) load_chunk(c);
    put_a(0);
  };
  fetch_rows(tile);
  asm volatile("s_waitcnt vmcnt(0)" ::: "memory");
  __syncthreads();
  while (true) {
    unsigned next_v = 0;
    if (tid == 256) next_v = atomicAdd(tile_ctr, 1u);
    unsigned base[4];
    s16x8_t hf[D / 16];
    s16x8_t wf[NF];
    f32x16_t bias_c;
    auto load_bias = [&](int at) {
#pragma unroll
      for (int q = 0; q < 4; ++q) {
        const f32x4_t bv = cst4(at + 8 * q);
        bias_c[4 * q + 0] = bv[0]; bias_c[4 * q + 1] = bv[1]; bias_c[4 * q + 2] = bv[2]; bias_c[4 * q + 3] = bv[3];
      }
    };
#pragma unroll
    for (int p = 0; p < PSTEPS; ++p) {
      sync_wait<true>();
      if (p % 2 == 0 && p / 2 + 1 < 6) put_a(p / 2 + 1);
      if (p == 0) load_chunk(6);
      if (p % 2 == 1 && p / 2 < 5) load_chunk(7 + p / 2);
      if (p == PSTEPS - 1) put_chunk(0);
      ring_advance(st);
    }
#pragma unroll
    for (int r = 0; r < 12; ++r) {
      sync_wait<true>();
      if (r + 1 < 12) put_chunk(r + 1);
    }
#pragma unroll
    for (int r = 0; r < 12; ++r) {
      sync_wait<true>();
      hf[2 * r] = *(lds_frag_ptr)(pbl + (r & 1) * PBH);
      hf[2 * r + 1] = *(lds_frag_ptr)(pbl + (r & 1) * PBH + 1024);
    }
    f32x16_t ga, gb = {};
    u32x4_t pk0 = {}, pk1 = {};
#pragma unroll
    for (int i = 0; i < 4; ++i) base[i] = lds0 + st.slot * SB + (aoff0 ^ (32 * i));
    auto put_gf = [&](int half) {
      *(lds_wu4_ptr)(pbl + half * PBH) = pk0;
      *(lds_wu4_ptr)(pbl + half * PBH + 1024) = pk1;
    };
    load_bias(C_B1);
    sync_wait<true>();
#pragma unroll
    for (int f = 0; f < NF; ++f) wf[f] = ld_frag(base, f);
#pragma unroll
    for (int j = 0; j < 12; ++j) {
      ga = mfma32<DT>(wf[j % NF], hf[j], j == 0 ? bias_c : ga);
      ring_gap<false, false>(st, base, wf, j, 0, 0);
      __builtin_amdgcn_sched_barrier(0);
    }
    ring_advance(st);
    f_step<DT, 1, false, false, false>(st, base, wf, hf, ga, bias_c, gb, pk1);
    for (int u = 1; u < UNITS - 1; u += 2) {
      load_bias(C_B1 + 32 * u);
      f_step<DT, 0, true, false, true>(st, base, wf, hf, gb, bias_c, ga, pk0);
      f_step<DT, 1, true, false, false>(st, base, wf, hf, gb, bias_c, ga, pk1);
      put_gf(0);
      load_bias(C_B1 + 32 * (u + 1));
      f_step<DT, 0, true, false, true>(st, base, wf, hf, ga, bias_c, gb, pk0);
      f_step<DT, 1, true, false, false>(st, base, wf, hf, ga, bias_c, gb, pk1);
      put_gf(1);
    }
    load_bias(C_B1 + 32 * (UNITS - 1));
    f_step<DT, 0, true, false, true>(st, base, wf, hf, gb, bias_c, ga, pk0);
    f_step<DT, 1, true, true, false>(st, base, wf, hf, gb, bias_c, ga, pk1);
    put_gf(0);
    sync_wait<true>();
    ring_advance(st);
#pragma unroll
    for (int r = 0; r < 16; r += 2) {
      const float v0 = gelu_poly(gb[r]), v1 = gelu_poly(gb[r + 1]);
      const unsigned w = pack2_h16<DT>(v0, v1);
      if (r < 8) pk0[r >> 1] = w; else pk1[(r - 8) >> 1] = w;
    }
    put_gf(1);
    sync_wait<true>(); ring_advance(st);
    sync_wait(); ring_advance(st);
    sync_wait(); ring_advance(st);
    if (tid == 256) *(lds_u32_ptr)nxt = next_v;
    asm volatile("s_waitcnt vmcnt(0) lgkmcnt(0)\n\ts_barrier" ::: "memory");
    const int next = __builtin_amdgcn_readfirstlane((int)*(lds_u32_ptr)nxt);
    if (next >= ntiles) break;
    tile = next;
    fetch_rows(tile);
  }
}

template <int DT>
__device__ __attribute__((noinline)) void run_x(Ctx c) {
  FX_ROLE_ENV;
  unsigned base[4];
  asm volatile("s_waitcnt vmcnt(0)" ::: "memory");
  __syncthreads();
  s16x8_t wf[NF];
  f32x16_t xacc[D / 32];
  while (true) {
    int ln = lane;
    asm volatile("" : "+v"(ln));
    {
#pragma unroll
      for (int ot = 0; ot < D / 32; ++ot)
#pragma unroll
        for (int q = 0; q < 4; ++q) {
          const f32x4_t bv = cst4(C_BP + 32 * ot + 8 * q);
          xacc[ot][4 * q + 0] = bv[0]; xacc[ot][4 * q + 1] = bv[1]; xacc[ot][4 * q + 2] = bv[2]; xacc[ot][4 * q + 3] = bv[3];
        }
#pragma unroll
      for (int i = 0; i < 4; ++i) base[i] = lds0 + st.slot * SB + (aoff0 ^ (32 * i));
      const unsigned af_rd = pbuf + (ln >> 5) * AF_H + (ln & 31) * 16;
      s16x8_t aa[2], ab[2];
      x_wait<-1, true>();
#pragma unroll
      for (int f = 0; f < NF; ++f) wf[f] = ld_frag(base, f);
      aa[0] = *(lds_frag_ptr)(af_rd + af_off(0));
      aa[1] = *(lds_frag_ptr)(af_rd + af_off(1));
      p_step<DT, -1, true, false>(st, base, wf, xacc, aa, ab, af_rd + af_off(2), af_rd + af_off(3));
      p_step<DT, -1, false, false>(st, base, wf, xacc, ab, aa, af_rd + af_off(4), af_rd + af_off(5));
#pragma unroll
      for (int p = 2; p < PSTEPS - 2; p += 2) {
        p_step<DT, WAIT0, false, false>(st, base, wf, xacc, aa, ab, af_rd + af_off(2 * p + 2), af_rd + af_off(2 * p + 3));
        p_step<DT, WAIT0, false, false>(st, base, wf, xacc, ab, aa, af_rd + af_off(2 * p + 4), af_rd + af_off(2 * p + 5));
      }
      p_step<DT, WAIT0, false, false>(st, base, wf, xacc, aa, ab, af_rd + af_off(2 * PSTEPS - 2), af_rd + af_off(2 * PSTEPS - 1));
      p_step<DT, WAIT0, false, true>(st, base, wf, xacc, ab, aa, 0, 0);
      const unsigned ch_rd = pbuf + (ln & 31) * STG_ROW + 16 * (ln >> 5);
#pragma unroll
      for (int r = 0; r < 12; ++r) {
        sync_wait<true>();
        f32x4_t xv[4];
#pragma unroll
        for (int g = 0; g < 4; ++g) xv[g] = *(lds_f4_ptr)(ch_rd + (r & 1) * PBH + 32 * g);
#pragma unroll
        for (int g = 0; g < 4; ++g)
#pragma unroll
          for (int e = 0; e < 4; ++e) xacc[r][4 * g + e] += xv[g][e];
      }
      float s = 0.f;
#pragma unroll
      for (int ot = 0; ot < D / 32; ++ot) {
#pragma unroll
        for (int g = 0; g < 4; ++g) s += (xacc[ot][4 * g + 0] + xacc[ot][4 * g + 1]) + (xacc[ot][4 * g + 2] + xacc[ot][4 * g + 3]);
        __builtin_amdgcn_sched_barrier(0);
      }
      {
        const auto sw = __builtin_amdgcn_permlane32_swap(__float_as_uint(s), __float_as_uint(s), false, false);
        s = __uint_as_float(sw[0]) + __uint_as_float(sw[1]);
      }
      const float mean = s / (float)D;
      float q = 0.f;
#pragma unroll
      for (int ot = 0; ot < D / 32; ++ot) {
#pragma unroll
        for (int r = 0; r < 16; ++r) { const float dv = xacc[ot][r] - mean; q += dv * dv; }
        __builtin_amdgcn_sched_barrier(0);
      }
      {
        const auto sw = __builtin_amdgcn_permlane32_swap(__float_as_uint(q), __float_as_uint(q), false, false);
        q = __uint_as_float(sw[0]) + __uint_as_float(sw[1]);
      }
      const float rstd = 1.0f / sqrtf(q / (float)D + ln_eps);
      float mean_p = mean;
      asm volatile("" : "+v"(mean_p));
      const unsigned hw_ = pbuf + ln * 16;
      f32x4_t gq[2][4], bq[2][4];
#pragma unroll
      for (int g = 0; g < 4; ++g) { gq[0][g] = cst4(C_G2 + 8 * g); bq[0][g] = cst4(C_E2 + 8 * g); }
#pragma unroll
      for (int ot = 0; ot < D / 32; ++ot) {
        if (ot + 1 < D / 32) {
#pragma unroll
          for (int g = 0; g < 4; ++g) { gq[(ot + 1) & 1][g] = cst4(C_G2 + 32 * (ot + 1) + 8 * g); bq[(ot + 1) & 1][g] = cst4(C_E2 + 32 * (ot + 1) + 8 * g); }
        }
#pragma unroll
        for (int k2 = 0; k2 < 2; ++k2) {
          u32x4_t pk;
#pragma unroll
          for (int g2_ = 0; g2_ < 2; ++g2_) {
            const int g = 2 * k2 + g2_;
            const f32x4_t gg = gq[ot & 1][g], bb = bq[ot & 1][g];
            pk[2 * g2_ + 0] = pack2_h16<DT>((xacc[ot][4 * g + 0] - mean_p) * rstd * gg[0] + bb[0], (xacc[ot][4 * g + 1] - mean_p) * rstd * gg[1] + bb[1]);
            pk[2 * g2_ + 1] = pack2_h16<DT>((xacc[ot][4 * g + 2] - mean_p) * rstd * gg[2] + bb[2], (xacc[ot][4 * g + 3] - mean_p) * rstd * gg[3] + bb[3]);
          }
          *(lds_wu4_ptr)(hw_ + (ot & 1) * PBH + k2 * 1024) = pk;
        }
        sync_wait<true>();
      }
    }
    s16x8_t gf[2];
    x_idle_step<WAIT0>(st); x_idle_step<WAIT0>(st); x_idle_step<WAIT0>(st);
    x_wait<WAIT0>();
    {
      const int g_next = ring_next(st), slot_free = ring_free(st);
#pragma unroll
      for (int i = 0; i < PIECES; ++i) ring_piece(st, i, g_next, slot_free);
      ring_advance(st);
#pragma unroll
      for (int i = 0; i < 4; ++i) base[i] = lds0 + st.slot * SB + HB + (aoff0 ^ (32 * i));
#pragma unroll
      for (int f = 0; f < NF; ++f) wf[f] = ld_frag(base, f);
    }
    const unsigned gfa = pbuf + ln * 16;
    for (int u = 0; u < UNITS - 2; u += 2) {
      x_step<DT, 0, false>(st, base, wf, xacc, gf, gfa);
      x_step<DT, 1, false>(st, base, wf, xacc, gf, gfa);
      x_step<DT, 0, false>(st, base, wf, xacc, gf, gfa + PBH);
      x_step<DT, 1, false>(st, base, wf, xacc, gf, gfa + PBH);
    }
    x_step<DT, 0, false>(st, base, wf, xacc, gf, gfa);
    x_step<DT, 1, false>(st, base, wf, xacc, gf, gfa);
    x_step<DT, 0, false>(st, base, wf, xacc, gf, gfa + PBH);
    x_step<DT, 1, true>(st, base, wf, xacc, gf, gfa + PBH);
    asm volatile("s_waitcnt vmcnt(0) lgkmcnt(0)\n\ts_barrier" ::: "memory");
    const int next = __builtin_amdgcn_readfirstlane((int)*(lds_u32_ptr)nxt);
    {
      const auto rxo = tile_rsrc(x, tile, D * 4);
      const auto rho = tile_rsrc(hout, tile, D * 2);
      int le = lane;
      asm volatile("" : "+v"(le));
      const unsigned stg_wr_e = pbuf + (le & 31) * STG_ROW + 16 * (le >> 5);
      const unsigned stg_wh = pbuf + (le & 31) * STG_ROW + 8 * (le >> 5);
      const unsigned stg_rd_e = pbuf + (le >> 3) * STG_ROW + (le & 7) * 16;
      const int xo_e = (rb * 32 + (le >> 3)) * (D * 4) + (le & 7) * 16;
      const int ho = (rb * 32 + (le >> 3)) * (D * 2) + (le & 7) * 16;
      float s = 0.f;
      {
        f32x4_t bvq[2][4];
#pragma unroll
        for (int g = 0; g < 4; ++g) bvq[0][g] = cst4(C_B2 + 8 * g);
#pragma unroll
        for (int ot = 0; ot < D / 32; ++ot) {
#pragma unroll
          for (int g = 0; g < 4; ++g) {
            const f32x4_t bv = bvq[ot & 1][g];
            f32x4_t v;
            v[0] = xacc[ot][4 * g + 0] + bv[0]; v[1] = xacc[ot][4 * g + 1] + bv[1];
            v[2] = xacc[ot][4 * g + 2] + bv[2]; v[3] = xacc[ot][4 * g + 3] + bv[3];
#pragma unroll
            for (int e = 0; e < 4; ++e) xacc[ot][4 * g + e] = v[e];
            *(lds_w4_ptr)(stg_wr_e + 32 * g) = v;
            s += (v[0] + v[1]) + (v[2] + v[3]);
          }
          __builtin_amdgcn_sched_barrier(0);
          f32x4_t rbk[4];
#pragma unroll
          for (int i = 0; i < 4; ++i) rbk[i] = *(lds_f4_ptr)(stg_rd_e + i * 8 * STG_ROW);
          if (ot + 1 < D / 32) {
#pragma unroll
            for (int g = 0; g < 4; ++g) bvq[(ot + 1) & 1][g] = cst4(C_B2 + 32 * (ot + 1) + 8 * g);
          }
          __builtin_amdgcn_sched_barrier(0);
#pragma unroll
          for (int i = 0; i < 4; ++i)
            __builtin_amdgcn_raw_buffer_store_b128(__builtin_bit_cast(u32x4_t, rbk[i]), rxo, xo_e + ot * 128, i * 8 * (D * 4), 0);
          __builtin_amdgcn_sched_barrier(0);
        }
      }
      if (hout) {
        {
          const auto sw = __builtin_amdgcn_permlane32_swap(__float_as_uint(s), __float_as_uint(s), false, false);
          s = __uint_as_float(sw[0]) + __uint_as_float(sw[1]);
        }
        const float mean = s / (float)D;
        float q = 0.f;
#pragma unroll
        for (int ot = 0; ot < D / 32; ++ot) {
#pragma unroll
          for (int r = 0; r < 16; ++r) { const float dv = xacc[ot][r] - mean; q += dv * dv; }
          __builtin_amdgcn_sched_barrier(0);
        }
        {
          const auto sw = __builtin_amdgcn_permlane32_swap(__float_as_uint(q), __float_as_uint(q), false, false);
          q = __uint_as_float(sw[0]) + __uint_as_float(sw[1]);
        }
        const float rstd = 1.0f / sqrtf(q / (float)D + ln_eps);
        float mean_p = mean;
        asm volatile("" : "+v"(mean_p));
        f32x4_t gq1[2][4], bq1[2][4];
#pragma unroll
        for (int g = 0; g < 4; ++g) { gq1[0][g] = cst4(C_G1 + 8 * g); bq1[0][g] = cst4(C_E1 + 8 * g); }
#pragma unroll
        for (int ot = 0; ot < D / 32; ++ot) {
          const int op = ot >> 1, o2 = ot & 1;
#pragma unroll
          for (int g = 0; g < 4; ++g) {
            const f32x4_t gg = gq1[ot & 1][g], bb = bq1[ot & 1][g];
            u32x2_t pk;
            pk[0] = pack2_h16<DT>((xacc[ot][4 * g + 0] - mean_p) * rstd * gg[0] + bb[0], (xacc[ot][4 * g + 1] - mean_p) * rstd * gg[1] + bb[1]);
            pk[1] = pack2_h16<DT>((xacc[ot][4 * g + 2] - mean_p) * rstd * gg[2] + bb[2], (xacc[ot][4 * g + 3] - mean_p) * rstd * gg[3] + bb[3]);
            *(lds_w2_ptr)(stg_wh + 64 * o2 + 16 * g) = pk;
          }
          __builtin_amdgcn_sched_barrier(0);
          [[maybe_unused]] f32x4_t rbk[4];
          if (o2) {
#pragma unroll
            for (int i = 0; i < 4; ++i) rbk[i] = *(lds_f4_ptr)(stg_rd_e + i * 8 * STG_ROW);
          }
          if (ot + 1 < D / 32) {
#pragma unroll
            for (int g = 0; g < 4; ++g) { gq1[(ot + 1) & 1][g] = cst4(C_G1 + 32 * (ot + 1) + 8 * g); bq1[(ot + 1) & 1][g] = cst4(C_E1 + 32 * (ot + 1) + 8 * g); }
          }
          __builtin_amdgcn_sched_barrier(0);
          if (o2) {
#pragma unroll
            for (int i = 0; i < 4; ++i)
              __builtin_amdgcn_raw_buffer_store_b128(__builtin_bit_cast(u32x4_t, rbk[i]), rho, ho + op * 128, i * 8 * (D * 2), 0);
            __builtin_amdgcn_sched_barrier(0);
          }
        }
      }
    }
    if (next >= ntiles) break;
    tile = next;
  }
}

template <int DT>
__global__ __launch_bounds__(512, 1) void tail_fx_kernel(const unsigned short* __restrict__ abuf, const unsigned short* __restrict__ wpk,
                                                         const float* __restrict__ bp, const float* __restrict__ g2, const float* __restrict__ e2,
                                                         const float* __restrict__ b1, const float* __restrict__ b2,
                                                         float* __restrict__ x, int64_t rows, const float* __restrict__ ln_g,
                                                         const float* __restrict__ ln_b, float ln_eps,
                                                         unsigned short* __restrict__ hout, int ntiles,
                                                         unsigned* __restrict__ tile_ctr) {
  __shared__ __attribute__((aligned(16))) char smem[LDS_BYTES];
  const int tid = threadIdx.x;
  const int lane = tid & 63, wave = __builtin_amdgcn_readfirstlane(tid >> 6);
  float* const cst = reinterpret_cast<float*>(smem + CONST_OFF);
  for (int i = tid; i < C_N; i += 512) {
    float v;
    if (i < C_B2) v = b1[i];
    else if (i < C_G1) v = b2[i - C_B2];
    else if (i < C_E1) v = ln_g ? ln_g[i - C_G1] : 1.f;
    else if (i < C_BP) v = ln_b ? ln_b[i - C_E1] : 0.f;
    else if (i < C_G2) v = bp[i - C_BP];
    else if (i < C_E2) v = g2[i - C_G2];
    else v = e2[i - C_E2];
    cst[i] = v;
  }
  const unsigned lds0 = (unsigned)(size_t)LDS_PTR(smem);
  const unsigned nxt = lds0 + NEXT_OFF;
  if (tid == 0) *(lds_u32_ptr)nxt = atomicAdd(tile_ctr, 1u);
  __syncthreads();
  const int tile = __builtin_amdgcn_readfirstlane((int)*(lds_u32_ptr)nxt);
  if (tile >= ntiles) return;
  if (wave < 4) {
    const i32x4_t rsrc = lds_dma_rsrc(wpk, (unsigned)(NSEQ * SB));
#pragma unroll
    for (int u = 0; u < AHEAD; ++u)
#pragma unroll
      for (int i = 0; i < PIECES; ++i)
        lds_dma16(rsrc, lds0 + wave * (PIECES * 1024) + u * SB + i * 1024, lane * 16, u * SB + wave * (PIECES * 1024) + i * 1024);
  }
  const Ctx c = {abuf, wpk, x, hout, tile_ctr, rows, ln_eps, ntiles, tile, lds0};
  if (wave >= 4) run_f<DT>(c);
  else run_x<DT>(c);
  asm volatile("s_waitcnt vmcnt(0)" ::: "memory");
}

}

extern "C" size_t vittf_block_tail_workspace_bytes(void) { return sizeof(unsigned); }

extern "C" int vittf_block_tail(const void* attn_out, const void* w_packed, const float* proj_b, const float* ln2_g,
                                const float* ln2_b, const float* b1, const float* b2, float* x, int64_t rows, int32_t d,
                                int32_t dtype, const float* ln_g, const float* ln_b, float ln_eps, void* h_out, void* tile_counter,
                                void* stream) {
  if (!attn_out || !w_packed || !proj_b || !ln2_g || !ln2_b || !b1 || !b2 || !x || rows <= 0) return VITTF_ERR_INVALID_ARG;
  if (d != D) return VITTF_ERR_INVALID_ARG;
  if ((ln_g || ln_b || h_out) && !(ln_g && ln_b && h_out)) return VITTF_ERR_INVALID_ARG;
  const int64_t tiles = (rows + 127) / 128;
  if (tiles > 0x7fffffff) return VITTF_ERR_INVALID_ARG;
  if ((((uintptr_t)attn_out | (uintptr_t)w_packed | (uintptr_t)x | (uintptr_t)h_out) & 15) != 0) return VITTF_ERR_INVALID_ARG;
  if (!tile_counter || ((uintptr_t)tile_counter & 3) != 0) return VITTF_ERR_INVALID_ARG;
  const int cus = vittf_current_cus();
  if (cus <= 0) return VITTF_ERR_NO_DEVICE;
  const unsigned grid = (unsigned)(tiles < cus ? tiles : cus);
  hipStream_t st = (hipStream_t)stream;
  unsigned* ctr = (unsigned*)tile_counter;
  if (hipMemsetAsync(ctr, 0, sizeof(unsigned), st) != hipSuccess) return VITTF_ERR_LAUNCH;
#define FX_LAUNCH(DTV)                                                                                               \
  hipLaunchKernelGGL((tail_fx_kernel<DTV>), dim3(grid), dim3(512), 0, st, (const unsigned short*)attn_out,           \
                     (const unsigned short*)w_packed, proj_b, ln2_g, ln2_b, b1, b2, x, rows, ln_g, ln_b, ln_eps,     \
                     (unsigned short*)h_out, (int)tiles, ctr)
  if (dtype == VITTF_BF16) FX_LAUNCH(VITTF_BF16);
  else if (dtype == VITTF_FP16) FX_LAUNCH(VITTF_FP16);
  else return VITTF_ERR_INVALID_ARG;
#undef FX_LAUNCH
  vittf_note_kernel(VITTF_KERNEL_MLP, "tail_fx_kernel");
  return vittf_check_launch();
}
```

vit-tf_amd/csrc/vittf_internal.h:

```cpp
#pragma once
#include "vittf_common.h"

static inline size_t align256(size_t x) { return (x + 255) & ~(size_t)255; }

static inline int64_t vittf_kfeat_out_bytes(int64_t rows, int32_t d, int32_t tokens, int32_t drop) {
  return (rows - rows / tokens * drop) * (int64_t)d * 2;
}

bool vittf_gemm_rows_covers(int32_t n, int32_t k, int64_t rows);
int vittf_gemm_rows(const void* a, const void* w, const float* bias, float* x, int64_t rows, int32_t n, int32_t k,
                    int32_t dtype, const float* ln_g, const float* ln_b, float ln_eps, void* h, hipStream_t st);

bool vittf_gemm_pp_covers(int32_t k, int32_t columns, const void* a, const void* w);
bool vittf_gemm_pp_covers_out(const void* out, int64_t kfeat_bytes);
int vittf_gemm_pp(const void* a, const void* w, const float* bias, void* out, int64_t rows, int32_t n, int32_t k,
                  int32_t epilogue, int32_t tokens, int32_t dtype, hipStream_t st);
int vittf_gemm_pp_kfeat_parts(const void* a, const void* w, const float* bias, int64_t rows, int32_t d, int32_t k,
                              int32_t tokens, int32_t n_reg, int32_t part_mask, void* const outs[3], int32_t dtype,
                              hipStream_t st, int32_t* taken);

int vittf_attention_pp64(const void* qkv, void* out, int32_t batch, int32_t tokens, int32_t heads, int32_t dtype,
                         hipStream_t st);

size_t vittf_sim_mfma_workspace_bytes(int32_t classes, int32_t annotations);
bool vittf_sim_mfma_applies(int32_t f, int32_t classes, int32_t total_a, const void* ws, size_t ws_bytes, const void* feat,
                            int64_t nvox);
int vittf_sim_mfma_maps(const unsigned short* feat, int32_t f, int64_t nvox, const float* qf, const int32_t* class_start_host,
                        int32_t classes, const float* voxel_norm, float* sim, unsigned* maxbits, void* ws, size_t ws_bytes,
                        hipStream_t st);
```

Before: 2349 slices/s.

## Fuse first LayerNorm into patch embed and skip final residual store

After: 2352 slices/s, median of 6. No clear change (+0.1%).

```diff
diff --git a/include/vittf.h b/include/vittf.h
--- a/include/vittf.h
+++ b/include/vittf.h
@@ -41,7 +41,8 @@
 enum {
   VITTF_CFG_SEPARATE_LN = 1,
   VITTF_CFG_UNSCALED_Q = 2,
-  VITTF_CFG_FP8_HEAD_SCALES = 4
+  VITTF_CFG_FP8_HEAD_SCALES = 4,
+  VITTF_CFG_SEPARATE_PASSES = 8
 };
 #define VITTF_MAX_REGISTER_TOKENS 8
 #define VITTF_TAIL_STEPS 112
@@ -139,6 +140,10 @@
                           const vittf_slice_view* view, int32_t slice0, int32_t batch, const float* reg_rows, int32_t n_reg,
                           float* tokens_out, void* stream);
 
+int vittf_patch_embed_ln(const vittf_vit_config* cfg, const vittf_vit_weights* w, const vittf_pos_embed* pos,
+                         const vittf_slice_view* view, int32_t slice0, int32_t batch, const float* reg_rows, int32_t n_reg,
+                         float* tokens_out, void* h_out, void* stream);
+
 int vittf_layernorm(const float* x, const float* g, const float* b, void* y, int64_t rows, int32_t d,
                     float eps, int32_t dtype, void* stream);
 
@@ -175,6 +180,12 @@
 int vittf_block_tail(const void* attn_out, const void* w_packed, const float* proj_b, const float* ln2_g, const float* ln2_b,
                      const float* b1, const float* b2, float* x, int64_t rows, int32_t d, int32_t dtype, const float* ln_g,
                      const float* ln_b, float ln_eps, void* h_out, void* tile_counter, void* stream);
+
+#define VITTF_TAIL_NO_X_STORE 1
+int vittf_block_tail_flags(const void* attn_out, const void* w_packed, const float* proj_b, const float* ln2_g,
+                           const float* ln2_b, const float* b1, const float* b2, float* x, int64_t rows, int32_t d, int32_t dtype,
+                           const float* ln_g, const float* ln_b, float ln_eps, void* h_out, void* tile_counter, int32_t flags,
+                           void* stream);
 
 int vittf_rope_qk(void* qkv, int64_t rows, int32_t tokens, int32_t prefix, int32_t heads, const vittf_rope_table* table,
                   int32_t dtype, void* stream);
diff --git a/vit-tf_amd/_lib.py b/vit-tf_amd/_lib.py
--- a/vit-tf_amd/_lib.py
+++ b/vit-tf_amd/_lib.py
@@ -15,7 +15,8 @@
                 ('dtype', C.c_int32), ('ln_eps', C.c_float), ('attention_fp8', C.c_int32), ('flags', C.c_int32)]
 
 
-CFG_SEPARATE_LN, CFG_UNSCALED_Q, CFG_FP8_HEAD_SCALES = 1, 2, 4
+CFG_SEPARATE_LN, CFG_UNSCALED_Q, CFG_FP8_HEAD_SCALES, CFG_SEPARATE_PASSES = 1, 2, 4, 8
+TAIL_NO_X_STORE = 1
 
 
 class VitWeights(C.Structure):
@@ -74,6 +75,8 @@
     'vittf_patch_embed': (C.c_int, [_P(VitConfig), _P(VitWeights), _P(PosEmbed), _P(SliceView), _i32, _i32, _vp, _vp]),
     'vittf_patch_embed_reg': (C.c_int, [_P(VitConfig), _P(VitWeights), _P(PosEmbed), _P(SliceView), _i32, _i32, _vp, _i32, _vp,
                                         _vp]),
+    'vittf_patch_embed_ln': (C.c_int, [_P(VitConfig), _P(VitWeights), _P(PosEmbed), _P(SliceView), _i32, _i32, _vp, _i32, _vp, _vp,
+                                       _vp]),
     'vittf_token_features': (C.c_int, [_vp, _vp, _vp, _vp, _i32, _i32, _i32, _i32, C.c_float, _vp]),
     'vittf_layernorm': (C.c_int, [_vp, _vp, _vp, _vp, _i64, _i32, C.c_float, _i32, _vp]),
     'vittf_gemm': (C.c_int, [_vp, _vp, _vp, _vp, _i64, _i32, _i32, _i32, _i32, _i32, _vp]),
@@ -82,6 +85,8 @@
     'vittf_gemm_residual_ln': (C.c_int, [_vp, _vp, _vp, _vp, _i64, _i32, _i32, _i32, _vp, _vp, C.c_float, _vp, _vp]),
     'vittf_block_tail_workspace_bytes': (_sz, []),
     'vittf_block_tail': (C.c_int, [_vp, _vp, _vp, _vp, _vp, _vp, _vp, _vp, _i64, _i32, _i32, _vp, _vp, C.c_float, _vp, _vp, _vp]),
+    'vittf_block_tail_flags': (C.c_int, [_vp, _vp, _vp, _vp, _vp, _vp, _vp, _vp, _i64, _i32, _i32, _vp, _vp, C.c_float, _vp, _vp, _i32,
+                                         _vp]),
     'vittf_gemm_as_workspace_bytes': (_sz, []),
     'vittf_gemm_as': (C.c_int, [_vp, _vp, _vp, _vp, _i64, _i32, _i32, _i32, _i32, _vp, _vp]),
     'vittf_rope_qk': (C.c_int, [_vp, _i64, _i32, _i32, _i32, _P(RopeTable), _i32, _vp]),
diff --git a/vit-tf_amd/csrc/engine.hip b/vit-tf_amd/csrc/engine.hip
--- a/vit-tf_amd/csrc/engine.hip
+++ b/vit-tf_amd/csrc/engine.hip
@@ -116,18 +116,22 @@
   void* O = base + lay.o;
   void* G = QKV;
 
-  int rc;
-  { ProfScope ps(VITTF_KERNEL_PATCH_EMBED, stream); rc = vittf_patch_embed_reg(cfg, w, pos, view, slice0, batch, reg_rows, n_reg, X, stream); }
-  if (rc) return rc;
   const size_t esz = 2;
   const bool res_ln = !(cfg->flags & VITTF_CFG_SEPARATE_LN) && (d == 384 || d == 768);
   const int pre = (cfg->flags & VITTF_CFG_UNSCALED_Q) ? 0 : 1;
   const bool fp8_rows = !(cfg->flags & VITTF_CFG_FP8_HEAD_SCALES) && cfg->attention_fp8 && pre && d >= 768 && d % 256 == 0;
   const bool tail = d == 384 && w->tail_packed && res_ln;
   const bool qkv_as = d == 384 && w->qkv_packed && !cfg->attention_fp8;
+  const bool passes = !(cfg->flags & VITTF_CFG_SEPARATE_PASSES) && !want_t;
+  const bool embed_ln = passes && tail && qkv_as && vittf_patch_embed_covers_ln(cfg, w, pos, reg_rows, n_reg, X, H);
+  int rc;
+  { ProfScope ps(VITTF_KERNEL_PATCH_EMBED, stream);
+    rc = embed_ln ? vittf_patch_embed_ln(cfg, w, pos, view, slice0, batch, reg_rows, n_reg, X, H, stream)
+                  : vittf_patch_embed_reg(cfg, w, pos, view, slice0, batch, reg_rows, n_reg, X, stream); }
+  if (rc) return rc;
   for (int l = 0; l < L; ++l) {
     const char* qkv_w = (const char*)w->qkv_w + (size_t)l * 3 * d * d * esz;
-    if (res_ln ? l == 0 : true) {
+    if (res_ln ? l == 0 && !embed_ln : true) {
       ProfScope ps(VITTF_KERNEL_LAYERNORM, stream);
       rc = vittf_layernorm(X, w->ln1_g + (size_t)l * d, w->ln1_b + (size_t)l * d, H, rows, d, cfg->ln_eps, dt, stream);
       if (rc) return rc;
@@ -161,11 +165,12 @@
         rc = vittf_attention(QKV, O, batch, tokens, cfg->heads, dt, pre, stream); }
     if (rc) return rc;
     if (tail) {
+      const int tail_flags = (passes && l == L - 2) ? VITTF_TAIL_NO_X_STORE : 0;
       ProfScope ps(VITTF_KERNEL_MLP, stream);
-      rc = vittf_block_tail(O, (const char*)w->tail_packed + (size_t)l * VITTF_TAIL_STEPS * 12288 * esz, w->proj_b + (size_t)l * d,
-                            w->ln2_g + (size_t)l * d, w->ln2_b + (size_t)l * d, w->fc1_b + (size_t)l * 4 * d,
-                            w->fc2_b + (size_t)l * d, X, rows, d, dt, next_g, next_b, cfg->ln_eps, H, base + lay.tile_ctr,
-                            stream);
+      rc = vittf_block_tail_flags(O, (const char*)w->tail_packed + (size_t)l * VITTF_TAIL_STEPS * 12288 * esz,
+                                  w->proj_b + (size_t)l * d, w->ln2_g + (size_t)l * d, w->ln2_b + (size_t)l * d,
+                                  w->fc1_b + (size_t)l * 4 * d, w->fc2_b + (size_t)l * d, X, rows, d, dt, next_g, next_b,
+                                  cfg->ln_eps, H, base + lay.tile_ctr, tail_flags, stream);
       if (rc) return rc;
       continue;
     }
diff --git a/vit-tf_amd/csrc/frontend.hip b/vit-tf_amd/csrc/frontend.hip
--- a/vit-tf_amd/csrc/frontend.hip
+++ b/vit-tf_amd/csrc/frontend.hip
@@ -1,4 +1,4 @@
-#include "vittf_common.h"
+#include "vittf_internal.h"
 
 namespace {
 
@@ -111,14 +111,61 @@
     for (int e = threadIdx.x; e < (1 + nreg) * d; e += blockDim.x) out_b[e] = e < d ? cls_pos0[e] : reg_rows[e - d];
 }
 
-constexpr int PEM_D = 384, PEM_K = 64, PEM_FRAGS = (PEM_D / 32) * (PEM_K / 16) * 2;
+constexpr int PEM_D = 384, PEM_K = 64, PEM_FRAGS = (PEM_D / 32) * (PEM_K / 16) * 2, PEM_OT = PEM_D / 32;
+
+template <typename F> __device__ __forceinline__ float row_tree_sum(F f4) {
+#pragma clang fp contract(off)
+  float t[16];
+#pragma unroll
+  for (int m = 0; m < 16; ++m) t[m] = ((0.f + f4(m)) + f4(m + 32)) + (0.f + f4(m + 16));
+#pragma unroll
+  for (int w = 8; w >= 1; w >>= 1)
+#pragma unroll
+    for (int m = 0; m < w; ++m) t[m] = t[m] + t[m + w];
+  return t[0] + __shfl_xor(t[0], 32);
+}
+
+template <int DT>
+__device__ __forceinline__ void row_layernorm(const f32x16_t (&v)[PEM_OT], int h, const float* __restrict__ g,
+                                              const float* __restrict__ b, float eps, unsigned short* __restrict__ yrow,
+                                              bool store) {
+#pragma clang fp contract(off)
+  const float s = row_tree_sum([&](int m) {
+    const int ot = m >> 2, q = 4 * (m & 3);
+    return (v[ot][q + 0] + v[ot][q + 1]) + (v[ot][q + 2] + v[ot][q + 3]);
+  });
+  const float mean = s / (float)PEM_D;
+  const float qs = row_tree_sum([&](int m) {
+    const int ot = m >> 2, q = 4 * (m & 3);
+    const float a0 = v[ot][q + 0] - mean, a1 = v[ot][q + 1] - mean, a2 = v[ot][q + 2] - mean, a3 = v[ot][q + 3] - mean;
+    return __builtin_fmaf(a0, a0, a1 * a1) + __builtin_fmaf(a2, a2, a3 * a3);
+  });
+  const float rstd = 1.0f / sqrtf(qs / (float)PEM_D + eps);
+  if (!store) return;
+#pragma unroll
+  for (int ot = 0; ot < PEM_OT; ++ot)
+#pragma unroll
+    for (int q = 0; q < 16; q += 4) {
+      const int c = 32 * ot + 2 * q + 4 * h;
+      const float4 gg = *reinterpret_cast<const float4*>(g + c), bb = *reinterpret_cast<const float4*>(b + c);
+      uint2 pk;
+      pk.x = pack2_h16<DT>(__builtin_fmaf((v[ot][q + 0] - mean) * rstd, gg.x, bb.x), __builtin_fmaf((v[ot][q + 1] - mean) * rstd, gg.y, bb.y));
+      pk.y = pack2_h16<DT>(__builtin_fmaf((v[ot][q + 2] - mean) * rstd, gg.z, bb.z), __builtin_fmaf((v[ot][q + 3] - mean) * rstd, gg.w, bb.w));
+      *reinterpret_cast<uint2*>(yrow + c) = pk;
+    }
+}
+
+template <int LN>
 __global__ __launch_bounds__(512, 1) void patch_embed_mfma_kernel(vittf_slice_view view, int slice0, int batch,
                                                                   const float* __restrict__ w_t, const float* __restrict__ bias,
                                                                   const float* __restrict__ cls_pos0,
                                                                   const float* __restrict__ patch_pos,
                                                                   float* __restrict__ tokens_out, int f0, int f1, int nreg,
-                                                                  const float* __restrict__ reg_rows) {
+                                                                  const float* __restrict__ reg_rows,
+                                                                  const float* __restrict__ ln_g, const float* __restrict__ ln_b,
+                                                                  float ln_eps, unsigned short* __restrict__ h_out) {
   __shared__ __attribute__((aligned(16))) unsigned short wlds[PEM_FRAGS * 512];
+  constexpr int TILES = LN >= 0 ? PEM_OT : PEM_OT / 2;
   const int tid = threadIdx.x, lane = tid & 63, wave = tid >> 6;
   const int h = lane >> 5, l31 = lane & 31;
   for (int it = tid; it < (PEM_FRAGS / 2) * 64; it += 512) {
@@ -173,43 +220,45 @@
     }
     float* orow = tokens_out + r * PEM_D;
     const float* prow = patch_pos + (int64_t)p * PEM_D;
+    f32x16_t acc[TILES];
 #pragma unroll 1
-    for (int pass = 0; pass < 2; ++pass) {
-      f32x16_t acc[6];
-#pragma unroll
-      for (int j = 0; j < 6; ++j)
+    for (int pass = 0; pass < PEM_OT / TILES; ++pass) {
+#pragma unroll
+      for (int j = 0; j < TILES; ++j)
 #pragma unroll
         for (int q = 0; q < 16; ++q) acc[j][q] = 0.f;
 #pragma unroll
       for (int s = 0; s < 4; ++s)
 #pragma unroll
-        for (int j = 0; j < 6; ++j) {
-          const int fr = (6 * pass + j) * 4 + s;
+        for (int j = 0; j < TILES; ++j) {
+          const int fr = (TILES * pass + j) * 4 + s;
           const s16x8_t ah = *reinterpret_cast<const s16x8_t*>(&wlds[((fr * 2 + 0) * 64 + lane) * 8]);
           const s16x8_t al = *reinterpret_cast<const s16x8_t*>(&wlds[((fr * 2 + 1) * 64 + lane) * 8]);
           acc[j] = mfma32<VITTF_FP16>(ah, bh[s], acc[j]);
           acc[j] = mfma32<VITTF_FP16>(al, bh[s], acc[j]);
           acc[j] = mfma32<VITTF_FP16>(ah, bl[s], acc[j]);
         }
-      if (valid) {
-#pragma unroll
-        for (int j = 0; j < 6; ++j)
+      if (valid || LN >= 0) {
+#pragma unroll
+        for (int j = 0; j < TILES; ++j)
 #pragma unroll
           for (int g = 0; g < 4; ++g) {
-            const int c = 32 * (6 * pass + j) + 8 * g + 4 * h;
-            float4 o;
+            const int c = 32 * (TILES * pass + j) + 8 * g + 4 * h;
+            float4 o = make_float4(0.f, 0.f, 0.f, 0.f);
             if (patch) {
               const float4 bv = *reinterpret_cast<const float4*>(bias + c);
               const float4 pv = *reinterpret_cast<const float4*>(prow + c);
               o.x = acc[j][4 * g + 0] + bv.x + pv.x; o.y = acc[j][4 * g + 1] + bv.y + pv.y;
               o.z = acc[j][4 * g + 2] + bv.z + pv.z; o.w = acc[j][4 * g + 3] + bv.w + pv.w;
-            } else {
+            } else if (valid) {
               o = *reinterpret_cast<const float4*>(crow + c);
             }
-            *reinterpret_cast<float4*>(orow + c) = o;
+            if (valid) *reinterpret_cast<float4*>(orow + c) = o;
+            if constexpr (LN >= 0) { acc[j][4 * g + 0] = o.x; acc[j][4 * g + 1] = o.y; acc[j][4 * g + 2] = o.z; acc[j][4 * g + 3] = o.w; }
           }
       }
     }
+    if constexpr (LN >= 0) row_layernorm<LN>(acc, h, ln_g, ln_b, ln_eps, h_out + r * PEM_D, valid);
   }
 }
 
@@ -336,9 +385,10 @@
   return vittf_check_launch();
 }
 
-extern "C" int vittf_patch_embed_reg(const vittf_vit_config* cfg, const vittf_vit_weights* w, const vittf_pos_embed* pos,
-                                     const vittf_slice_view* view, int32_t slice0, int32_t batch, const float* reg_rows,
-                                     int32_t n_reg, float* tokens_out, void* stream) {
+static int patch_embed(const vittf_vit_config* cfg, const vittf_vit_weights* w, const vittf_pos_embed* pos,
+                       const vittf_slice_view* view, int32_t slice0, int32_t batch, const float* reg_rows, int32_t n_reg,
+                       float* tokens_out, const float* ln_g, const float* ln_b, float ln_eps, int32_t ln_dtype, void* h_out,
+                       void* stream) {
   if (!cfg || !w || !pos || !view || !tokens_out || batch <= 0 || slice0 < 0) return VITTF_ERR_INVALID_ARG;
   if (n_reg < 0 || n_reg > VITTF_MAX_REGISTER_TOKENS || (n_reg > 0 && !reg_rows)) return VITTF_ERR_INVALID_ARG;
   if (!w->pe_w_t || !w->pe_b || !pos->cls_plus_pos0 || !pos->patch_pos || !view->vol || !view->minmax)
@@ -356,11 +406,19 @@
     const int cus = vittf_current_cus();
     if (cus <= 0) return VITTF_ERR_NO_DEVICE;
     const int64_t ntile = ((int64_t)batch * (f0 * f1 + 1 + n_reg) + 255) / 256;
+    const dim3 grid((unsigned)(ntile < cus ? ntile : cus));
     vittf_note_kernel(VITTF_KERNEL_PATCH_EMBED, "patch_embed_mfma_kernel");
-    hipLaunchKernelGGL(patch_embed_mfma_kernel, dim3((unsigned)(ntile < cus ? ntile : cus)), dim3(512), 0, st, *view, slice0, batch,
-                       w->pe_w_t, w->pe_b, pos->cls_plus_pos0, pos->patch_pos, tokens_out, f0, f1, n_reg, reg_rows);
+#define PEM_LAUNCH(LN)                                                                                                           \
+  hipLaunchKernelGGL((patch_embed_mfma_kernel<LN>), grid, dim3(512), 0, st, *view, slice0, batch, w->pe_w_t, w->pe_b,           \
+                     pos->cls_plus_pos0, pos->patch_pos, tokens_out, f0, f1, n_reg, reg_rows, ln_g, ln_b, ln_eps,               \
+                     (unsigned short*)h_out)
+    if (!h_out) PEM_LAUNCH(-1);
+    else if (ln_dtype == VITTF_BF16) PEM_LAUNCH(VITTF_BF16);
+    else PEM_LAUNCH(VITTF_FP16);
+#undef PEM_LAUNCH
     return vittf_check_launch();
   }
+  if (h_out) return VITTF_ERR_INVALID_ARG;
   if (cfg->embed_dim == PEM_D && p == PE14_P && aligned) {
     const int cus = vittf_current_cus();
     if (cus <= 0) return VITTF_ERR_NO_DEVICE;
@@ -389,6 +447,30 @@
   return vittf_check_launch();
 }
 
+extern "C" int vittf_patch_embed_reg(const vittf_vit_config* cfg, const vittf_vit_weights* w, const vittf_pos_embed* pos,
+                                     const vittf_slice_view* view, int32_t slice0, int32_t batch, const float* reg_rows,
+                                     int32_t n_reg, float* tokens_out, void* stream) {
+  return patch_embed(cfg, w, pos, view, slice0, batch, reg_rows, n_reg, tokens_out, nullptr, nullptr, 0.f, 0, nullptr, stream);
+}
+
+bool vittf_patch_embed_covers_ln(const vittf_vit_config* cfg, const vittf_vit_weights* w, const vittf_pos_embed* pos,
+                                 const float* reg_rows, int32_t n_reg, const float* tokens_out, const void* h_out) {
+  if (!cfg || !w || !pos) return false;
+  return cfg->embed_dim == PEM_D && cfg->patch == 8 &&
+         (((uintptr_t)w->pe_b | (uintptr_t)pos->cls_plus_pos0 | (uintptr_t)pos->patch_pos | (uintptr_t)tokens_out | (uintptr_t)h_out |
+           (uintptr_t)w->ln1_g | (uintptr_t)w->ln1_b | (n_reg > 0 ? (uintptr_t)reg_rows : 0)) & 15) == 0;
+}
+
+extern "C" int vittf_patch_embed_ln(const vittf_vit_config* cfg, const vittf_vit_weights* w, const vittf_pos_embed* pos,
+                                    const vittf_slice_view* view, int32_t slice0, int32_t batch, const float* reg_rows,
+                                    int32_t n_reg, float* tokens_out, void* h_out, void* stream) {
+  if (!cfg || !w || !h_out || !w->ln1_g || !w->ln1_b) return VITTF_ERR_INVALID_ARG;
+  if (cfg->dtype != VITTF_BF16 && cfg->dtype != VITTF_FP16) return VITTF_ERR_INVALID_ARG;
+  if (!vittf_patch_embed_covers_ln(cfg, w, pos, reg_rows, n_reg, tokens_out, h_out)) return VITTF_ERR_INVALID_ARG;
+  return patch_embed(cfg, w, pos, view, slice0, batch, reg_rows, n_reg, tokens_out, (const float*)w->ln1_g, (const float*)w->ln1_b,
+                     cfg->ln_eps, cfg->dtype, h_out, stream);
+}
+
 extern "C" int vittf_patch_embed(const vittf_vit_config* cfg, const vittf_vit_weights* w, const vittf_pos_embed* pos,
                                  const vittf_slice_view* view, int32_t slice0, int32_t batch, float* tokens_out,
                                  void* stream) {
diff --git a/vit-tf_amd/csrc/tail_fx.hip b/vit-tf_amd/csrc/tail_fx.hip
--- a/vit-tf_amd/csrc/tail_fx.hip
+++ b/vit-tf_amd/csrc/tail_fx.hip
@@ -366,7 +366,7 @@
   }
 }
 
-template <int DT>
+template <int DT, bool STORE_X>
 __device__ __attribute__((noinline)) void run_x(Ctx c) {
   FX_ROLE_ENV;
   unsigned base[4];
@@ -503,7 +503,7 @@
       const int xo_e = (rb * 32 + (le >> 3)) * (D * 4) + (le & 7) * 16;
       const int ho = (rb * 32 + (le >> 3)) * (D * 2) + (le & 7) * 16;
       float s = 0.f;
-      {
+      if constexpr (STORE_X) {
         f32x4_t bvq[2][4];
 #pragma unroll
         for (int g = 0; g < 4; ++g) bvq[0][g] = cst4(C_B2 + 8 * g);
@@ -532,6 +532,28 @@
 #pragma unroll
           for (int i = 0; i < 4; ++i)
             __builtin_amdgcn_raw_buffer_store_b128(__builtin_bit_cast(u32x4_t, rbk[i]), rxo, xo_e + ot * 128, i * 8 * (D * 4), 0);
+          __builtin_amdgcn_sched_barrier(0);
+        }
+      } else {
+        f32x4_t bvq[2][4];
+#pragma unroll
+        for (int g = 0; g < 4; ++g) bvq[0][g] = cst4(C_B2 + 8 * g);
+#pragma unroll
+        for (int ot = 0; ot < D / 32; ++ot) {
+          if (ot + 1 < D / 32) {
+#pragma unroll
+            for (int g = 0; g < 4; ++g) bvq[(ot + 1) & 1][g] = cst4(C_B2 + 32 * (ot + 1) + 8 * g);
+          }
+#pragma unroll
+          for (int g = 0; g < 4; ++g) {
+            const f32x4_t bv = bvq[ot & 1][g];
+            f32x4_t v;
+            v[0] = xacc[ot][4 * g + 0] + bv[0]; v[1] = xacc[ot][4 * g + 1] + bv[1];
+            v[2] = xacc[ot][4 * g + 2] + bv[2]; v[3] = xacc[ot][4 * g + 3] + bv[3];
+#pragma unroll
+            for (int e = 0; e < 4; ++e) xacc[ot][4 * g + e] = v[e];
+            s += (v[0] + v[1]) + (v[2] + v[3]);
+          }
           __builtin_amdgcn_sched_barrier(0);
         }
       }
@@ -594,14 +616,14 @@
   }
 }
 
-template <int DT>
-__global__ __launch_bounds__(512, 1) void tail_fx_kernel(const unsigned short* __restrict__ abuf, const unsigned short* __restrict__ wpk,
-                                                         const float* __restrict__ bp, const float* __restrict__ g2, const float* __restrict__ e2,
-                                                         const float* __restrict__ b1, const float* __restrict__ b2,
-                                                         float* __restrict__ x, int64_t rows, const float* __restrict__ ln_g,
-                                                         const float* __restrict__ ln_b, float ln_eps,
-                                                         unsigned short* __restrict__ hout, int ntiles,
-                                                         unsigned* __restrict__ tile_ctr) {
+#define FX_KERNEL_ARGS                                                                                                   \
+  const unsigned short *__restrict__ abuf, const unsigned short *__restrict__ wpk, const float *__restrict__ bp,         \
+      const float *__restrict__ g2, const float *__restrict__ e2, const float *__restrict__ b1, const float *__restrict__ b2, \
+      float *__restrict__ x, int64_t rows, const float *__restrict__ ln_g, const float *__restrict__ ln_b, float ln_eps,  \
+      unsigned short *__restrict__ hout, int ntiles, unsigned *__restrict__ tile_ctr
+
+template <int DT, bool STORE_X>
+__device__ __forceinline__ void tail_fx_body(FX_KERNEL_ARGS) {
   __shared__ __attribute__((aligned(16))) char smem[LDS_BYTES];
   const int tid = threadIdx.x;
   const int lane = tid & 63, wave = __builtin_amdgcn_readfirstlane(tid >> 6);
@@ -633,18 +655,28 @@
   }
   const Ctx c = {abuf, wpk, x, hout, tile_ctr, rows, ln_eps, ntiles, tile, lds0};
   if (wave >= 4) run_f<DT>(c);
-  else run_x<DT>(c);
+  else run_x<DT, STORE_X>(c);
   asm volatile("s_waitcnt vmcnt(0)" ::: "memory");
 }
 
+template <int DT> __global__ __launch_bounds__(512, 1) void tail_fx_kernel(FX_KERNEL_ARGS) {
+  tail_fx_body<DT, true>(abuf, wpk, bp, g2, e2, b1, b2, x, rows, ln_g, ln_b, ln_eps, hout, ntiles, tile_ctr);
+}
+template <int DT> __global__ __launch_bounds__(512, 1) void tail_hx_kernel(FX_KERNEL_ARGS) {
+  tail_fx_body<DT, false>(abuf, wpk, bp, g2, e2, b1, b2, x, rows, ln_g, ln_b, ln_eps, hout, ntiles, tile_ctr);
+}
+#undef FX_KERNEL_ARGS
+
 }
 
 extern "C" size_t vittf_block_tail_workspace_bytes(void) { return sizeof(unsigned); }
 
-extern "C" int vittf_block_tail(const void* attn_out, const void* w_packed, const float* proj_b, const float* ln2_g,
-                                const float* ln2_b, const float* b1, const float* b2, float* x, int64_t rows, int32_t d,
-                                int32_t dtype, const float* ln_g, const float* ln_b, float ln_eps, void* h_out, void* tile_counter,
-                                void* stream) {
+extern "C" int vittf_block_tail_flags(const void* attn_out, const void* w_packed, const float* proj_b, const float* ln2_g,
+                                      const float* ln2_b, const float* b1, const float* b2, float* x, int64_t rows, int32_t d,
+                                      int32_t dtype, const float* ln_g, const float* ln_b, float ln_eps, void* h_out,
+                                      void* tile_counter, int32_t flags, void* stream) {
+  if (flags & ~VITTF_TAIL_NO_X_STORE) return VITTF_ERR_INVALID_ARG;
+  if ((flags & VITTF_TAIL_NO_X_STORE) && !h_out) return VITTF_ERR_INVALID_ARG;
   if (!attn_out || !w_packed || !proj_b || !ln2_g || !ln2_b || !b1 || !b2 || !x || rows <= 0) return VITTF_ERR_INVALID_ARG;
   if (d != D) return VITTF_ERR_INVALID_ARG;
   if ((ln_g || ln_b || h_out) && !(ln_g && ln_b && h_out)) return VITTF_ERR_INVALID_ARG;
@@ -658,14 +690,23 @@
   hipStream_t st = (hipStream_t)stream;
   unsigned* ctr = (unsigned*)tile_counter;
   if (hipMemsetAsync(ctr, 0, sizeof(unsigned), st) != hipSuccess) return VITTF_ERR_LAUNCH;
-#define FX_LAUNCH(DTV)                                                                                               \
-  hipLaunchKernelGGL((tail_fx_kernel<DTV>), dim3(grid), dim3(512), 0, st, (const unsigned short*)attn_out,           \
+  const bool store_x = !(flags & VITTF_TAIL_NO_X_STORE);
+#define FX_LAUNCH(KERNEL, DTV)                                                                                       \
+  hipLaunchKernelGGL((KERNEL<DTV>), dim3(grid), dim3(512), 0, st, (const unsigned short*)attn_out,                   \
                      (const unsigned short*)w_packed, proj_b, ln2_g, ln2_b, b1, b2, x, rows, ln_g, ln_b, ln_eps,     \
                      (unsigned short*)h_out, (int)tiles, ctr)
-  if (dtype == VITTF_BF16) FX_LAUNCH(VITTF_BF16);
-  else if (dtype == VITTF_FP16) FX_LAUNCH(VITTF_FP16);
+  if (dtype == VITTF_BF16) { if (store_x) FX_LAUNCH(tail_fx_kernel, VITTF_BF16); else FX_LAUNCH(tail_hx_kernel, VITTF_BF16); }
+  else if (dtype == VITTF_FP16) { if (store_x) FX_LAUNCH(tail_fx_kernel, VITTF_FP16); else FX_LAUNCH(tail_hx_kernel, VITTF_FP16); }
   else return VITTF_ERR_INVALID_ARG;
 #undef FX_LAUNCH
-  vittf_note_kernel(VITTF_KERNEL_MLP, "tail_fx_kernel");
+  vittf_note_kernel(VITTF_KERNEL_MLP, store_x ? "tail_fx_kernel" : "tail_hx_kernel");
   return vittf_check_launch();
 }
+
+extern "C" int vittf_block_tail(const void* attn_out, const void* w_packed, const float* proj_b, const float* ln2_g,
+                                const float* ln2_b, const float* b1, const float* b2, float* x, int64_t rows, int32_t d,
+                                int32_t dtype, const float* ln_g, const float* ln_b, float ln_eps, void* h_out, void* tile_counter,
+                                void* stream) {
+  return vittf_block_tail_flags(attn_out, w_packed, proj_b, ln2_g, ln2_b, b1, b2, x, rows, d, dtype, ln_g, ln_b, ln_eps, h_out,
+                                tile_counter, 0, stream);
+}
diff --git a/vit-tf_amd/csrc/vittf_internal.h b/vit-tf_amd/csrc/vittf_internal.h
--- a/vit-tf_amd/csrc/vittf_internal.h
+++ b/vit-tf_amd/csrc/vittf_internal.h
@@ -19,6 +19,9 @@
                               int32_t tokens, int32_t n_reg, int32_t part_mask, void* const outs[3], int32_t dtype,
                               hipStream_t st, int32_t* taken);
 
+bool vittf_patch_embed_covers_ln(const vittf_vit_config* cfg, const vittf_vit_weights* w, const vittf_pos_embed* pos,
+                                 const float* reg_rows, int32_t n_reg, const float* tokens_out, const void* h_out);
+
 int vittf_attention_pp64(const void* qkv, void* out, int32_t batch, int32_t tokens, int32_t heads, int32_t dtype,
                          hipStream_t st);
 
```
